# DeepakSridhar/fgdm

Hardware: AMD Instinct MI355X
Metric: 512x512 images/sec @ 50 DDIM steps, seg-ControlNet+CFG (higher is better)
Workload: dtype f16

## Files before the change

fgdm_amd/_lib.py:

```python
import ctypes as C
import os

HERE = os.path.dirname(os.path.abspath(__file__))
LIB_PATH = os.path.join(HERE, 'libfgdm_hip.so')

MAX_LEVELS = 8
MAX_CONTROLNETS = 4

FLAG_USE_ORIGINAL = 1
FLAG_ONLY_MID_CONTROL = 2
FLAG_NO_CONTROL = 4
FLAG_CFG_PAIRS = 8

ACT_NONE, ACT_SILU, ACT_RELU, ACT_GEGLU, ACT_QGELU = 0, 1, 2, 3, 4
OUT_F16, OUT_F32, OUT_F32_NCHW, OUT_F16_T = 0, 1, 2, 3
STRIDE2_PAD_BR = -2


class FgdmConfig(C.Structure):
    _fields_ = [
        ('in_channels', C.c_int32), ('out_channels', C.c_int32), ('model_channels', C.c_int32),
        ('num_res_blocks', C.c_int32), ('n_levels', C.c_int32), ('channel_mult', C.c_int32 * MAX_LEVELS),
        ('n_attention_resolutions', C.c_int32), ('attention_resolutions', C.c_int32 * MAX_LEVELS),
        ('num_heads', C.c_int32), ('context_dim', C.c_int32), ('use_adapter', C.c_int32),
# ... 3 lines not shown
        ('clip_layers', C.c_int32), ('clip_width', C.c_int32), ('clip_heads', C.c_int32), ('clip_mlp', C.c_int32),
        ('clip_vocab', C.c_int32), ('clip_max_len', C.c_int32),
        ('n_extra_adapters', C.c_int32),
        ('vae_encoder', C.c_int32),
    ]


class FgdmConfig2(FgdmConfig):
    _fields_ = [('num_head_channels', C.c_int32), ('use_linear_in_transformer', C.c_int32)]


class FgdmDdimParams(C.Structure):
    _fields_ = [('struct_size', C.c_int64)] + [(name, C.c_void_p) for name in (
        'x', 'cond', 'uncond', 'timesteps', 'alphas', 'alphas_prev', 'sqrt_one_minus_alphas', 'control_scales', 'sigmas',
        'cfg_scales', 'step_noise', 'mask', 'x0', 'q_noise', 'sqrt_alphas_cumprod_t', 'sqrt_one_minus_alphas_cumprod_t',
        'log_steps', 'x_inter_out', 'pred_x0_out')] + [('cfg_scale', C.c_float)] + [(name, C.c_int32) for name in (
            'S', 'B', 'H', 'W', 'flags', 'n_log', 'reserved0')]


class FgdmPlmsParams(C.Structure):
    _fields_ = [('struct_size', C.c_int64)] + [(name, C.c_void_p) for name in (
        'x', 'cond', 'uncond', 'timesteps', 'alphas', 'alphas_prev', 'sqrt_one_minus_alphas', 'control_scales', 'mask', 'x0',
        'q_noise', 'sqrt_alphas_cumprod_t', 'sqrt_one_minus_alphas_cumprod_t', 'log_steps', 'x_inter_out', 'pred_x0_out')] + [
            ('cfg_scale', C.c_float)] + [(name, C.c_int32) for name in ('S', 'B', 'H', 'W', 'flags', 'n_log', 'reserved0')]


class FgdmDpmppParams(C.Structure):
    _fields_ = [('struct_size', C.c_int64)] + [(name, C.c_void_p) for name in (
        'x', 'cond', 'uncond', 'control_scales', 't_float', 'inv_alpha', 'neg_sigma_over_alpha', 'update_kind', 'c1', 'cm0',
        'cm1')] + [('cfg_scale', C.c_float)] + [(name, C.c_int32) for name in (
            'n_eval', 'B', 'H', 'W', 'flags', 'reserved0', 'reserved1')]


class FgdmDpmSolverParams(C.Structure):
    _fields_ = [('struct_size', C.c_int64)] + [(name, C.c_void_p) for name in (
        'x', 'cond', 'uncond', 'control_scales', 't_float', 'conv_x', 'conv_e', 'slot', 'nterms', 'plane', 'coef', 'dest')] + [
            ('cfg_scale', C.c_float)] + [(name, C.c_int32) for name in ('n_eval', 'B', 'H', 'W', 'flags', 'reserved0', 'reserved1')]


class FgdmAncestralParams(C.Structure):
    _fields_ = [('struct_size', C.c_int64)] + [(name, C.c_void_p) for name in (
        'x', 'cond', 'timesteps', 'sqrt_recip_alphas_cumprod', 'sqrt_recipm1_alphas_cumprod', 'posterior_mean_coef1',
        'posterior_mean_coef2', 'std', 'step_noise', 'control_scales', 'mask', 'x0', 'q_noise', 'sqrt_alphas_cumprod_t',
        'sqrt_one_minus_alphas_cumprod_t', 'log_steps', 'x_inter_out')] + [(name, C.c_int32) for name in (
            'S', 'B', 'H', 'W', 'flags', 'n_log', 'reserved0', 'reserved1')]


class FgdmDdimEncodeParams(C.Structure):
    _fields_ = [('struct_size', C.c_int64)] + [(name, C.c_void_p) for name in (
        'x', 'cond', 'uncond', 'timesteps', 'cx', 'ce', 'control_scales', 'log_steps', 'x_inter_out')] + [
            ('cfg_scale', C.c_float)] + [(name, C.c_int32) for name in ('S', 'B', 'H', 'W', 'flags', 'n_log', 'reserved0')]


class FgdmAttentionCapture(C.Structure):
    _fields_ = [('struct_size', C.c_int64), ('tokens', C.POINTER(C.c_int32)), ('block_mask', C.c_uint32)] + [
        (name, C.c_int32) for name in ('n_tokens', 'rows', 'mode', 'batch', 'latent_h', 'latent_w', 'reserved0')]


ATTENTION_CAPTURE_MAX_KEYS = 256
CAPTURE_ROWS = {'all': 0, 'cond': 1, 'uncond': 2}
CAPTURE_MODES = {'sum': 0, 'last': 1}
DPMPP_FIRST, DPMPP_SECOND = 1, 2
DPM_PLANE_BASE, DPM_PLANE_HIST0, DPM_PLANE_M, DPM_DEST_STATE, DPM_DEST_EVAL = 0, 1, 4, 1, 2
PLMS_PROBE, PLMS_FINISH_FIRST, PLMS_MULTISTEP = 0, 1, 2

_p = C.c_void_p
_f = C.c_float
_i = C.c_int
_i64 = C.c_int64

SIGNATURES = {
    'fgdm_create': (_i, [C.POINTER(FgdmConfig), _i, C.POINTER(_p)]),
    'fgdm_destroy': (None, [_p]),
    'fgdm_last_error': (C.c_char_p, [_p]),
    'fgdm_param_count': (_i, [C.POINTER(FgdmConfig)]),
    'fgdm_param_info': (_i, [C.POINTER(FgdmConfig), _i, C.c_char_p, _i, C.POINTER(_i64), C.POINTER(_i)]),
    'fgdm_load_tensor': (_i, [_p, C.c_char_p, _p, _i, C.POINTER(_i64), _i]),
    'fgdm_finalize_weights': (_i, [_p]),
    'fgdm_set_hint': (_i, [_p, _i, _p, _i, _i, _i, _p]),
    'fgdm_set_concat': (_i, [_p, _p, _i, _i, _i, _i, _p]),
    'fgdm_set_adapter_conds': (_i, [_p, _p, _i, _i, _i, _i, _p]),
    'fgdm_set_context': (_i, [_p, _p, _i, _p]),
    'fgdm_apply_model': (_i, [_p, _p, _p, _p, _p, _p, _p, _i, _i, _i, _i, _p, _p]),
    'fgdm_clip_encode': (_i, [_p, _p, _i, _i, _p, _p]),
    'fgdm_clip_encode_skip': (_i, [_p, _p, _i, _i, _i, _p, _p]),
    'fgdm_set_context_tokens': (_i, [_p, _i]),
    'fgdm_get_context_tokens': (_i, [_p]),
    'fgdm_attention_capture_set': (_i, [_p, C.POINTER(FgdmAttentionCapture)]),
    'fgdm_attention_capture_reset': (_i, [_p, _p]),
    'fgdm_attention_capture_info': (_i, [_p, _i, C.POINTER(_i64), C.POINTER(C.c_int32)]),
    'fgdm_attention_capture_block_size': (_i, [_p, _i, C.POINTER(C.c_int32), C.POINTER(C.c_int32)]),
    'fgdm_attention_capture_read': (_i, [_p, _i, _p, _p]),
    'fgdm_run_block': (_i, [_p, C.c_char_p, _p, _i, _p, _i, _p, _p, _i, _i, _i, _p, _i64, C.POINTER(_i64), _p]),
    'fgdm_vae_decode': (_i, [_p, _p, _i, _i, _i, _f, _p, _p]),
    'fgdm_vae_encode': (_i, [_p, _p, _i, _i, _i, _p, _p]),
    'fgdm_unfold': (_i, [_p] + [_i] * 10 + [_p, _p]),
    'fgdm_fold_weighted': (_i, [_p, _p, _p] + [_i] * 9 + [_p, _p]),
    'fgdm_vae_decode_patches': (_i, [_p, _p, _i, _i, _i, _f] + [_i] * 5 + [_p, _p, _i, _p, _p]),
    'fgdm_apply_model_patches': (_i, [_p, _p, _p, _p, _p] + [_i] * 7 + [_p, _p, _i, _i, _p, _p]),
    'fgdm_posterior_sample': (_i, [_p, _p, _f, _p, _i, _i, _i, _p]),
    'fgdm_image_to_uint8': (_i, [_p, _i, _i, _i, _i, _i, _p, _p]),
    'fgdm_resize_linear_uint8': (_i, [_p, _i, _i, _i, _i, _i, _i, _p, _p]),
    'fgdm_uint8_to_hint': (_i, [_p, _i, _i, _i, _i, _p, _p]),
    'fgdm_controlnet': (_i, [_p, _i, _p, _p, _p, _i, _i, _i, _p, _i64, _p]),
    'fgdm_ddim_step': (_i, [_p, _p, _p, _f, _f, _f, _f, _f, _p, _p, _p, _p, _i64, _p]),
    'fgdm_plms_combine': (_i, [_p, _p, _p, _p, _i, _p, _i64, _p]),
    'fgdm_axpby': (_i, [_p, _f, _p, _f, _p, _i64, _p]),
    'fgdm_mask_blend': (_i, [_p, _p, _p, _p, _i64, _p]),
    'fgdm_ancestral_step': (_i, [_p, _p, _f, _f, _f, _f, _f, _p, _p, _i64, _p]),
    'fgdm_sample_ddim': (_i, [_p, _p, _p, _p, _f, _i, C.POINTER(_i64), C.POINTER(_f), C.POINTER(_f), C.POINTER(_f),
                              _p, _i, _i, _i, _i, _p]),
    'fgdm_sample_ddim_ex': (_i, [_p, C.POINTER(FgdmDdimParams), _p]),
    'fgdm_op_ddim_loop_step': (_i, [_p, _p, _p, _f, _f, _f, _f, _f, _p, _p, _p, _p, _f, _f, _p, _p, _p, _p, _p, _i64, _p]),
    'fgdm_sample_plms': (_i, [_p, C.POINTER(FgdmPlmsParams), _p]),
    'fgdm_sample_dpmpp': (_i, [_p, C.POINTER(FgdmDpmppParams), _p]),
    'fgdm_op_plms_loop_step': (_i, [_p, _p, _p, _f, _i, _i, _p, _p, _p, _p, _f, _f, _f, _p, _p, _p, _f, _f, _p, _p, _p, _p, _p,
                                    _i64, _p]),
    'fgdm_op_dpmpp_loop_step': (_i, [_p, _p, _p, _f, _f, _f, _p, _i, _f, _f, _f, _p, _p, _p, _p, _i64, _p]),
    'fgdm_sample_dpm_solver': (_i, [_p, C.POINTER(FgdmDpmSolverParams), _p]),
    'fgdm_op_dpm_program_step': (_i, [_p, _p, _p, _f, _f, _f, _p, _p, _p, _p, _i, _i, _p, _p, _p, _p, _p, _i64, _p]),
    'fgdm_sample_ancestral': (_i, [_p, C.POINTER(FgdmAncestralParams), _p]),
    'fgdm_ddim_encode': (_i, [_p, C.POINTER(FgdmDdimEncodeParams), _p]),
    'fgdm_op_ancestral_loop_step': (_i, [_p, _p, _f, _f, _f, _f, _f, _p, _p, _p, _p, _f, _f, _p, _p, _p, _i64, _p]),
    'fgdm_op_invert_loop_step': (_i, [_p, _p, _p, _f, _f, _f, _p, _p, _p, _p, _i64, _p]),
    'fgdm_profile_begin': (_i, [_p, _i]),
    'fgdm_profile_end': (_i, [_p, C.POINTER(C.c_double)]),
    'fgdm_workspace_stats': (_i, [_p, C.POINTER(_i64), C.POINTER(_i64)]),
    'fgdm_launch_stats': (_i, [_p, C.POINTER(_i64), C.POINTER(_i64), C.POINTER(_i64)]),
    'fgdm_replay_plan': (_i, [_i, _p, _p, _p, _p, _i, _i, _p, _i, _p]),
    'fgdm_op_conv2d': (_i, [_p, _i, _p, _i, _p, _p, _p, _p, _i, _i, _i, _i, _i, _i, _i, _i, _f, _p, _p]),
    'fgdm_op_linear': (_i, [_p, _p, _p, _p, _i, _i, _i, _i, _i, _i, _i, _p, _p]),
    'fgdm_debug_force_igemm_cfg': (_i, [_i]),
    'fgdm_bench_igemm': (_i, [_i] * 13 + [C.POINTER(_f)]),
    'fgdm_op_linear_ln_linear': (_i, [_p] * 8 + [_i] * 5 + [_p, _p, C.POINTER(_i), _p]),
    'fgdm_bench_norm': (_i, [_i] * 7 + [C.POINTER(_f)]),
    'fgdm_bench_attention': (_i, [_i] * 6 + [C.POINTER(_f)]),
    'fgdm_bench_attention_maps': (_i, [_i] * 7 + [C.POINTER(_f)]),
    'fgdm_bench_ff': (_i, [_i] * 4 + [C.POINTER(_f)]),
    'fgdm_op_groupnorm': (_i, [_p, _i, _p, _i, _i, _i, _p, _p, _f, _i, _p, _p]),
    'fgdm_op_layernorm': (_i, [_p, _i, _i, _p, _p, _f, _p, _p]),
    'fgdm_op_attention': (_i, [_p, _i, _p, _i, _p, _i, _p, _i, _i, _i, _i, _i, _i, _p]),
    'fgdm_op_attention_ex': (_i, [_p, _i, _p, _i, _p, _i, _p, _i, _i, _i, _i, _i, _i, _i, _p]),
    'fgdm_debug_last_attention_kernel': (_i, []),
    'fgdm_op_cross_attention_maps': (_i, [_p, _i, _p, _i, _p, _i, _p, _i, _p, _i, _i, _i, _i, _i, _i, _p]),
    'fgdm_op_small_attention': (_i, [_p, _i, _i, _i, _p, _i, _i, _i, _i, _i, _i, _p]),
    'fgdm_op_vae_attention': (_i, [_p, _p, _p, _p, _i, _i, _i, _p]),
    'fgdm_op_softmax_rows': (_i, [_p, _p, _i, _i, _p]),
    'fgdm_op_nchw_to_nhwc': (_i, [_p, _p, _i, _i, _i, _i, _p]),
    'fgdm_op_nhwc_to_nchw': (_i, [_p, _p, _i, _i, _i, _p]),
    'fgdm_op_pack_xcat': (_i, [_p, _p, _i, _i, _i, _i, _i, _i, _p, _p]),
    'fgdm_op_avgpool2': (_i, [_p, _p, _i, _i, _i, _i, _p]),
    'fgdm_op_transpose_pad': (_i, [_p, _p, _i, _i, _i, _i, _p]),
    'fgdm_op_timestep_embed': (_i, [_p, _p, _p, _i, _i, _i, _p]),
    'fgdm_op_add_f16': (_i, [_p, _p, _p, _i64, _p]),
    'fgdm_op_ln_qkv': (_i, [_p] * 6 + [_i] * 5 + [_p, _p, _p]),
}

_lib = None


def load():
    global _lib
    if _lib is not None:
        return _lib
    try:
        import torch
# ... 14 lines not shown
```

fgdm_amd/csrc/engine.hip:

```cpp
#include "model.h"
#include "knobs.h"
#include "replay.h"

#include <algorithm>
#include <array>
#include <cmath>
#include <cstdlib>
#include <cstdio>
#include <cstring>
#include <map>
#include <memory>
#include <string>
#include <unordered_map>
#include <vector>

namespace {

struct Arena {
    struct Blk { char* p; size_t sz; bool free; };
    std::vector<std::vector<Blk>> slabs;
    std::vector<char*> bases;
    size_t slab_bytes = (size_t)4 << 30;
    size_t in_use = 0, peak = 0;
    bool scoped = false;
    std::vector<void*> live;
    void begin_scope() { scoped = true; live.clear(); }
    void end_scope(bool failed) {
        if (failed) { std::vector<void*> l; l.swap(live); scoped = false; for (void* p : l) release(p); }
        scoped = false;
        live.clear();
    }

    ~Arena() { for (char* b : bases) (void)hipFree(b); }
    void* alloc(size_t bytes) {
        bytes = (bytes + 255) & ~(size_t)255;
        if (bytes == 0) bytes = 256;
        for (auto& s : slabs)
            for (size_t i = 0; i < s.size(); ++i)
                if (s[i].free && s[i].sz >= bytes) {
                    if (s[i].sz > bytes) {
                        Blk rest{s[i].p + bytes, s[i].sz - bytes, true};
                        s[i].sz = bytes;
                        s.insert(s.begin() + i + 1, rest);
                    }
                    s[i].free = false;
                    in_use += bytes;
                    peak = std::max(peak, in_use);
                    if (scoped) live.push_back(s[i].p);
                    return s[i].p;
                }
        const size_t sz = std::max(slab_bytes, bytes);
        char* base = nullptr;
        if (hipMalloc(&base, sz) != hipSuccess) return nullptr;
        bases.push_back(base);
        slabs.push_back({Blk{base, sz, true}});
        return alloc(bytes);
    }
    void release(void* p) {
        if (!p) return;
        if (scoped) { auto it = std::find(live.begin(), live.end(), p); if (it != live.end()) { *it = live.back(); live.pop_back(); } }
        for (auto& s : slabs)
            for (size_t i = 0; i < s.size(); ++i)
                if (s[i].p == p && !s[i].free) {
                    s[i].free = true;
                    in_use -= s[i].sz;
                    if (i + 1 < s.size() && s[i + 1].free) { s[i].sz += s[i + 1].sz; s.erase(s.begin() + i + 1); }
                    if (i > 0 && s[i - 1].free) { s[i - 1].sz += s[i].sz; s.erase(s.begin() + i); }
                    return;
                }
    }
};

enum ProfClass { PC_IGEMM = 0, PC_ATTN = 1, PC_NORM = 2, PC_ELEM = 3, PC_COUNT = 4 };
struct Prof final : LaunchTimer {
    bool on = false;
    std::vector<hipEvent_t> pool;
    size_t used = 0;
    struct Rec { int cls; size_t e0, e1; double w; char tag[56]; };
    std::vector<Rec> recs;
    double work[PC_COUNT] = {0, 0, 0, 0};
    double bytes[PC_COUNT] = {0, 0, 0, 0};
    hipEvent_t get() {
        if (used == pool.size()) { hipEvent_t e; if (hipEventCreate(&e) != hipSuccess) return nullptr; pool.push_back(e); }
        return pool[used++];
    }
// ... 39 lines not shown
    struct CtxKV { Tensor k, vt; };
    std::unordered_map<const Layer*, CtxKV> ctx_cache;
    int ctx_B = 0, ctx_T = 0;
    int ctx_tokens = 77;
    struct CapPlane { int block = 0, heads = 0, h = 0, w = 0; float* acc = nullptr; };
    struct Capture {
        bool on = false, capturing = false;
        int rows_sel = 0, mode = 0, Tk = 0;
        int B = 0, H = 0, W = 0;
        int row0 = 0, rows = 0, n_evals = 0;
        std::vector<int> tokens;
        int* tok_dev = nullptr;
        float* head_planes = nullptr;
        std::vector<const Layer*> order;
        std::unordered_map<const Layer*, CapPlane> planes;
    } cap;
    void capture_free() {
        for (auto& kv : cap.planes) { (void)hipFree(kv.second.acc); kv.second.acc = nullptr; }
        (void)hipFree(cap.tok_dev); (void)hipFree(cap.head_planes);
        cap.tok_dev = nullptr; cap.head_planes = nullptr;
        cap.B = cap.H = cap.W = 0;
    }
    void capture_off() { capture_free(); cap = Capture{}; }
    size_t capture_plane_floats(const CapPlane& p) const { return (size_t)cap.rows * p.h * p.w * cap.tokens.size(); }
    int capture_alloc(int B, int H, int W) {
        capture_free();
        const bool half = cap.rows_sel != FGDM_CAPTURE_ROWS_ALL;
        if (half && (B & 1)) return fail(FGDM_ERR_STATE, "attention capture: the conditional / unconditional half of an odd batch");
        cap.rows = half ? B / 2 : B;
        cap.row0 = cap.rows_sel == FGDM_CAPTURE_ROWS_COND ? B / 2 : 0;
        int h = H, w = W;
        size_t scratch = 0;
        auto walk = [&](const Block& blk) -> int {
            for (const Layer& l : blk) {
                if (l.type == L_DOWN) { h = (h + 1) / 2; w = (w + 1) / 2; }
                if (l.type == L_UP) { h *= 2; w *= 2; }
                auto it = l.type == L_ATTN ? cap.planes.find(&l) : cap.planes.end();
                if (it == cap.planes.end()) continue;
                CapPlane& p = it->second;
                p.h = h; p.w = w; p.heads = l.heads;
                scratch = std::max(scratch, attention_capture_plane_floats(B, l.heads, h * w, cap.Tk));
            }
            return FGDM_OK;
        };
        CHK0(for_each_block(unet, false, walk));
        bool ok = hipMalloc(&cap.tok_dev, cap.tokens.size() * sizeof(int)) == hipSuccess &&
                  hipMemcpy(cap.tok_dev, cap.tokens.data(), cap.tokens.size() * sizeof(int), hipMemcpyHostToDevice) == hipSuccess &&
                  hipMalloc(&cap.head_planes, scratch * sizeof(float)) == hipSuccess;
        for (auto& kv : cap.planes) {
            const size_t bytes = capture_plane_floats(kv.second) * sizeof(float);
            ok = ok && hipMalloc(&kv.second.acc, bytes) == hipSuccess && hipMemset(kv.second.acc, 0, bytes) == hipSuccess;
        }
        if (!ok) { capture_free(); return fail(FGDM_ERR_NOMEM, "hipMalloc (attention capture)"); }
        cap.B = B; cap.H = H; cap.W = W;
        cap.n_evals = 0;
        return FGDM_OK;
    }
    int capture_begin(int B, int H, int W) {
        if (cap.Tk != ctx_tokens) return fail(FGDM_ERR_STATE, "attention capture: the context token count changed after the plan was set");
        if (!cap.B) CHK0(capture_alloc(B, H, W));
        if (B != cap.B || H != cap.H || W != cap.W)
            return fail(FGDM_ERR_STATE, "attention capture: this evaluation's batch or latent size is not the one the accumulators were made for");
        cap.capturing = true;
        ++cap.n_evals;
        return FGDM_OK;
    }
    Tensor ccat;
    Arena arena;
    half_t* zero = nullptr;
    int cur_comp = -1;
    bool ln_fold = true;
    hipStream_t s = nullptr;
    std::vector<std::unique_ptr<Arena>> cn_arena;
    Arena* ar = &arena;
    hipStream_t s2 = nullptr;
    hipEvent_t ev_fork = nullptr, ev_join = nullptr;
    bool twin_streams = false;
    bool pair_launch = true;
    int group_max = FGDM_MAX_GROUP;
    bool gn_group = true;
    ReplayStats replay_stats;
    struct Deferred { const GemmW* w; Tensor src; int idx; float scale; Arena* owner; };
    Prof prof;

    const ParamSlot* slot(const std::string& name) {
        auto it = params.find(name);
        if (it == params.end() || !it->second.loaded) { err = "parameter not loaded: " + name; return nullptr; }
        return &it->second;
    }
    template <typename T> T* upload(const std::vector<T>& h) {
        T* d = nullptr;
        if (hipMalloc(&d, std::max<size_t>(h.size() * sizeof(T), 256)) != hipSuccess) return nullptr;
        if (hipMemcpy(d, h.data(), h.size() * sizeof(T), hipMemcpyHostToDevice) != hipSuccess) return nullptr;
        comps[cur_comp].allocs.push_back(d);
        return d;
    }
    int pack_rows(GemmW& g, const std::vector<std::pair<const float*, int>>& srcs, int K_src, int K,
                  const std::vector<int>& kmap, const std::vector<const float*>& biases, bool geglu,
                  const std::vector<float>& src_scale = {}, const float* ln_gamma = nullptr, const float* ln_beta = nullptr) {
        int N = 0;
        for (auto& s : srcs) N += s.second;
        const size_t npad = igemm_npad(N);
        std::vector<half_t> w(npad * (size_t)K, (half_t)0);
        std::vector<float> bias(npad, 0.f), lnu(ln_gamma ? npad : 0, 0.f);
        std::vector<const float*> rowp(N);
        std::vector<float> bflat(N, 0.f), rscale(N, 1.f);
        int r = 0;
        for (size_t si = 0; si < srcs.size(); ++si)
            for (int i = 0; i < srcs[si].second; ++i, ++r) {
                rowp[r] = srcs[si].first + (size_t)i * K_src;
                if (si < biases.size() && biases[si]) bflat[r] = biases[si][i];
                if (si < src_scale.size()) rscale[r] = src_scale[si];
            }
        for (int pr = 0; pr < N; ++pr) {
            int sr = pr;
            if (geglu) {
                const int grp = pr >> 6, within = pr & 63;
                sr = within < 32 ? grp * 32 + within : N / 2 + grp * 32 + (within - 32);
            }
            const float* src = rowp[sr];
            const float rs = rscale[sr];
            half_t* dst = w.data() + (size_t)pr * K;
            if (ln_gamma) {
                double us = 0.0, cs = 0.0;
                for (int k = 0; k < K; ++k) {
                    dst[k] = (half_t)(src[k] * rs * ln_gamma[k]);
                    us += (double)(float)dst[k];
                    cs += (double)ln_beta[k] * (double)(src[k] * rs);
                }
                lnu[pr] = (float)us;
                bias[pr] = (float)((double)(bflat[sr] * rs) + cs);
                continue;
            }
            if (kmap.empty()) for (int k = 0; k < K; ++k) dst[k] = (half_t)(src[k] * rs);
            else for (int k = 0; k < K; ++k) if (kmap[k] >= 0) dst[k] = (half_t)(src[kmap[k]] * rs);
            bias[pr] = bflat[sr] * rs;
        }
        g.N = N; g.K = K; g.k_real = K_src;
        g.w = upload(w);
        g.bias = upload(bias);
        g.ln_u = ln_gamma ? upload(lnu) : nullptr;
        if (ln_gamma && !kmap.empty()) return fail(FGDM_ERR_ARG, "LayerNorm fold: plain Linear weights only");
        return (g.w && g.bias && (!ln_gamma || g.ln_u)) ? FGDM_OK : fail(FGDM_ERR_NOMEM, "hipMalloc failed while packing weights");
    }
    int pack_linear(GemmW& g, const std::string& pre, bool has_bias, bool geglu = false, float wscale = 1.f,
                    const std::string& ln = std::string()) {
        const ParamSlot* w = slot(pre + ".weight");
        if (!w) return FGDM_ERR_STATE;
        const ParamSlot *lg = nullptr, *lb = nullptr;
        if (!ln.empty()) { lg = slot(ln + ".weight"); lb = slot(ln + ".bias"); if (!lg || !lb) return FGDM_ERR_STATE; }
        const ParamSlot* b = has_bias ? slot(pre + ".bias") : nullptr;
        if (has_bias && !b) return FGDM_ERR_STATE;
        const int N = (int)w->shape[0], K = (int)(w->numel() / w->shape[0]);
        if (K & 63) return fail(FGDM_ERR_ARG, "linear K not a multiple of 64: " + pre);
        if (lg && (int)lg->numel() != K) return fail(FGDM_ERR_ARG, "LayerNorm fold: width mismatch for " + pre);
        return pack_rows(g, {{w->host.data(), N}}, K, K, {}, {b ? b->host.data() : nullptr}, geglu, {wscale},
                         lg ? lg->host.data() : nullptr, lb ? lb->host.data() : nullptr);
    }
    int pack_stack(GemmW& g, const std::vector<std::string>& pres, bool has_bias, const std::vector<float>& scales = {},
                   const std::string& ln = std::string()) {
        const ParamSlot *lg = nullptr, *lb = nullptr;
        if (!ln.empty()) { lg = slot(ln + ".weight"); lb = slot(ln + ".bias"); if (!lg || !lb) return FGDM_ERR_STATE; }
        std::vector<std::pair<const float*, int>> srcs;
        std::vector<const float*> biases;
        int K = 0;
        for (auto& pre : pres) {
// ... 382 lines not shown
          int rc;
          auto cp = cap.capturing ? cap.planes.find(&l) : cap.planes.end();
          if (cp != cap.planes.end()) {
              const CapPlane& p = cp->second;
              if (B != cap.B || T != p.h * p.w || Tk != cap.Tk) return fail(FGDM_ERR_STATE, "attention capture: block shape differs from the plan's");
              rc = attention_capture_launch(q2.p, C, k2.p, C, v2t.p, Tkp, a.p, C, B, l.heads, T, Tk, d, 1, cap.head_planes, s);
              if (rc == FGDM_OK)
                  rc = attention_maps_reduce(cap.head_planes, p.acc, l.heads, T, Tk, cap.row0, cap.rows, cap.tok_dev, (int)cap.tokens.size(),
                                             cap.mode == FGDM_CAPTURE_SUM, s);
          } else {
              rc = attention_launch(q2.p, C, k2.p, C, v2t.p, Tkp, a.p, C, B, l.heads, T, Tk, d, 1, s);
          }
          prof.end(s);
          if (rc != FGDM_OK) return fail(rc, "attention launch failed"); }
        tfree(q2);
        if (!cached) { tfree(k2); tfree(v2t); }
        { Epi e; e.resid = h2.p; e.ld_res = C; if (ln_fold) e.stats = &s3; CHK(linear(l.o2, a, e, &h)); }
        tfree(a); tfree(h2);
        if (!ln_fold) CHK(lnorm(l.ln3, h, &nrm));
        { Epi e; if (ln_fold) e.ln = &s3; e.act = ACT_GEGLU; CHK(linear(l.ffp, ln_fold ? h : nrm, e, &f)); }
        if (s3.p) ar->release(s3.p);
        if (nrm.p) tfree(nrm);
        { Epi e; e.resid = h.p; e.ld_res = C; CHK(linear(l.ffo, f, e, &h2)); }
        tfree(f); tfree(h);
        { Epi e; e.resid = x.p; e.ld_res = C; CHK(linear(l.pout, h2, e, out)); }
        tfree(h2);
        if (x_full.p) tfree(x_full);
        return FGDM_OK;
    }

    int dup_rows(const Tensor& h, Tensor* full) {
        *full = talloc(2 * h.B, h.H, h.W, h.C);
        if (!full->p) return fail(FGDM_ERR_NOMEM, "workspace");
        const size_t bytes = h.numel() * sizeof(half_t);
        CHK(dcopy(full->p, h.p, bytes));
        CHK(dcopy((char*)full->p + bytes, h.p, bytes));
        return FGDM_OK;
    }
    int block_fwd_shared(const Block& blk, Tensor xh, bool own_x, const EmbCtx& ec, const Tensor& ctx16, Tensor* out) {
        Tensor cur = xh;
        bool own = own_x, full = false;
        for (size_t j = 0; j < blk.size(); ++j) {
            const Layer& l = blk[j];
            Tensor nxt;
            switch (l.type) {
                case L_CONV: CHK(conv3(l.conv, cur, nullptr, 1, false, Epi{}, &nxt)); break;
                case L_RES: CHK(res_fwd(l, cur, nullptr, ec, &nxt)); break;
                case L_ATTN: CHK(attn_fwd(l, cur, ctx16, &nxt, !full)); full = true; break;
                case L_DOWN: CHK(conv3(l.conv, cur, nullptr, 2, false, Epi{}, &nxt)); break;
                case L_UP: CHK(conv3(l.conv, cur, nullptr, 1, true, Epi{}, &nxt)); break;
            }
            if (own) tfree(cur);
            cur = nxt;
            own = true;
        }
        if (!full) { Tensor f; CHK(dup_rows(cur, &f)); if (own) tfree(cur); cur = f; }
        *out = cur;
        return FGDM_OK;
    }

    int block_fwd(const Block& blk, Tensor x, bool own_x, const Tensor* x1, const EmbCtx& ec, const Tensor& ctx16,
                  const half_t* conv_resid, Tensor* out) {
        Tensor cur = x;
        bool own = own_x;
        for (size_t j = 0; j < blk.size(); ++j) {
            const Layer& l = blk[j];
            Tensor nxt;
            switch (l.type) {
                case L_CONV: { Epi e; if (conv_resid) { e.resid = conv_resid; e.ld_res = l.cout; }
                               CHK(conv3(l.conv, cur, nullptr, 1, false, e, &nxt)); break; }
                case L_RES: CHK(res_fwd(l, cur, j == 0 ? x1 : nullptr, ec, &nxt)); break;
                case L_ATTN: CHK(attn_fwd(l, cur, ctx16, &nxt)); break;
                case L_DOWN: CHK(conv3(l.conv, cur, nullptr, 2, false, Epi{}, &nxt)); break;
                case L_UP: CHK(conv3(l.conv, cur, nullptr, 1, true, Epi{}, &nxt)); break;
            }
            if (own) tfree(cur);
            cur = nxt;
            own = true;
        }
        *out = cur;
        return FGDM_OK;
    }

    int embed(Net& n, const int64_t* t, const float* tf, int B, float** emb_all) {
        const int mc = cfg.model_channels;
        Tensor te = talloc(1, 1, B, mc), e1, e2;
        if (!te.p) return fail(FGDM_ERR_NOMEM, "workspace");
        if (timestep_embed(t, tf, te.p, B, mc, B, s) != FGDM_OK) return fail(FGDM_ERR_HIP, "timestep_embed");
        { Epi e; e.act = ACT_SILU; e.rps = 1; CHK(linear(n.time0, te, e, &e1)); }
        { Epi e; e.act = ACT_SILU; e.rps = 1; CHK(linear(n.time2, e1, e, &e2)); }
        *emb_all = (float*)ar->alloc((size_t)B * n.emb_total * sizeof(float));
        if (!*emb_all) return fail(FGDM_ERR_NOMEM, "workspace");
        { Epi e; e.out_kind = OUT_F32; e.out = *emb_all; e.ld_out = n.emb_total; e.rps = 1; CHK(linear(n.emb_all, e2, e, nullptr)); }
        tfree(te); tfree(e1); tfree(e2);
        return FGDM_OK;
    }

    int adapter_fwd(Net& n, const Tensor& x4, Tensor feats[4]) { return adapter_run(n.ad_conv_in, n.ad_body, x4, feats); }
    int adapter_run(const GemmW& conv_in, const std::vector<AdapterBlk>& body, const Tensor& x4, Tensor feats[4]) {
        Tensor cur;
        CHK(conv3(conv_in, x4, nullptr, 1, false, Epi{}, &cur));
        auto drop = [&](Tensor& t) {
            for (int f = 0; f < 4; ++f) if (feats[f].p == t.p) return;
            tfree(t);
        };
        for (size_t k = 0; k < body.size(); ++k) {
            const AdapterBlk& b = body[k];
            if (b.down) {
                Tensor p = talloc(cur.B, cur.H / 2, cur.W / 2, cur.C);
                if (!p.p) return fail(FGDM_ERR_NOMEM, "workspace");
                if (avgpool2(cur.p, p.p, cur.B, cur.H, cur.W, cur.C, s) != FGDM_OK)
                    return fail(FGDM_ERR_ARG, "avgpool2: latent size must be divisible by 8 for the adapter");
                drop(cur);
                cur = p;
            }
            if (b.ic != b.oc) { Tensor y; CHK(linear(b.in_conv, cur, Epi{}, &y)); drop(cur); cur = y; }
            Tensor h, y;
            { Epi e; e.act = ACT_RELU; CHK(conv3(b.b1, cur, nullptr, 1, false, e, &h)); }
            { Epi e; e.resid = cur.p; e.ld_res = cur.C; CHK(linear(b.b2, h, e, &y)); }
            tfree(h);
            drop(cur);
            cur = y;
            if (k % 2 == 1) feats[k / 2] = cur;
        }
        return FGDM_OK;
    }

    void drop_adapter_conds() {
        for (Tensor& t : unet.xad_sum) { if (t.p) (void)hipFree(t.p); t = Tensor{}; }
        unet.xad_valid = false;
    }
    int set_adapter_conds(const float* const* conds, int nc, int B, int H, int W) {
        if (!finalized) return fail(FGDM_ERR_STATE, "weights not finalized");
        Net& n = unet;
        drop_adapter_conds();
        if (nc == 0) return FGDM_OK;
        if (nc < 0 || nc > (int)n.xad_body.size() || !conds) return fail(FGDM_ERR_ARG, "more conds than extra adapters (n_extra_adapters)");
        if (B <= 0 || (H & 7) || (W & 7)) return fail(FGDM_ERR_ARG, "latent size must be divisible by 8 for the adapter");
        for (int kk = 0; kk < nc; ++kk) {
            Tensor c4 = talloc(B, H, W, 4), f[4];
            if (!c4.p) return fail(FGDM_ERR_NOMEM, "workspace");
            if (nchw_f32_to_nhwc_f16(conds[kk], c4.p, B, 4, H * W, 4, s) != FGDM_OK) return fail(FGDM_ERR_HIP, "layout kernel");
            CHK(adapter_run(n.xad_conv_in[kk], n.xad_body[kk], c4, f));
            tfree(c4);
            for (int i = 0; i < 4; ++i) {
                Tensor& acc = n.xad_sum[i];
                if (kk == 0) {
                    acc = f[i];
                    if (hipMalloc(&acc.p, acc.numel() * sizeof(half_t)) != hipSuccess) return fail(FGDM_ERR_NOMEM, "hipMalloc (adapter cache)");
                    HIP_TRY(hipMemcpyAsync(acc.p, f[i].p, acc.numel() * sizeof(half_t), hipMemcpyDeviceToDevice, s));
                } else if (add_f16(acc.p, f[i].p, acc.p, acc.numel(), s) != FGDM_OK) {
                    return fail(FGDM_ERR_HIP, "add kernel");
                }
                tfree(f[i]);
            }
        }
        n.xad_valid = true;
        return FGDM_OK;
    }

    int time_adapter_fwd(Net& n, const Tensor& x4, const EmbCtx& ec, Tensor feats[4]) {
        Tensor cur;
        CHK(conv3(n.ad_conv_in, x4, nullptr, 1, false, Epi{}, &cur));
        for (size_t k = 0; k < n.tad_body.size(); ++k) {
            Tensor y;
            CHK(res_fwd(n.tad_body[k], cur, nullptr, ec, &y));
            bool keep = false;
            for (int f = 0; f < 4; ++f) if (feats[f].p == cur.p) keep = true;
            if (!keep) tfree(cur);
            cur = y;
            if (k % 2 == 1) feats[k / 2] = cur;
        }
        return FGDM_OK;
    }

    int run_block(const std::string& prefix, const float* x, int C, const float* x_skip, int Cs, const float* emb,
                  const float* ctx, int B, int H, int W, float* out, int64_t cap, int64_t* out_numel) {
        if (!finalized) return fail(FGDM_ERR_STATE, "weights not finalized");
        if (B <= 0 || H <= 0 || W <= 0 || C <= 0) return fail(FGDM_ERR_ARG, "bad shape");
// ... 60 lines not shown
            if (f32_to_f16(ctx, ctx16.p, ctx16.numel(), s) != FGDM_OK) return fail(FGDM_ERR_HIP, "convert kernel");
        }
        float* emb_all = nullptr;
        if (needs_emb) {
            const int temb = 4 * cfg.model_channels;
            Tensor e2 = talloc(1, 1, B, temb);
            emb_all = (float*)ar->alloc((size_t)B * net->emb_total * sizeof(float));
            if (!e2.p || !emb_all) return fail(FGDM_ERR_NOMEM, "workspace");
            if (silu_f32_to_f16(emb, e2.p, e2.numel(), s) != FGDM_OK) return fail(FGDM_ERR_HIP, "silu kernel");
            { Epi e; e.out_kind = OUT_F32; e.out = emb_all; e.ld_out = net->emb_total; e.rps = 1; CHK(linear(net->emb_all, e2, e, nullptr)); }
            tfree(e2);
        }
        EmbCtx ec{emb_all, net->emb_total};
        Tensor y;
        CHK(block_fwd(*blk, xin, false, x_skip ? &xsk : nullptr, ec, ctx16, nullptr, &y));
        CHK(emit(y, off));
        tfree(y); tfree(xin);
        if (xsk.p) tfree(xsk);
        if (ctx16.p) tfree(ctx16);
        if (emb_all) ar->release(emb_all);
        if (out_numel) *out_numel = off;
        return FGDM_OK;
    }

    int ensure_device() {
        if (device_ready) return FGDM_OK;
        if (hipSetDevice(device) != hipSuccess) return fail(FGDM_ERR_HIP, "hipSetDevice failed (no GPU?)");
        if (hipMalloc(&zero, 4096) != hipSuccess || hipMemset(zero, 0, 4096) != hipSuccess) return fail(FGDM_ERR_HIP, "hipMalloc failed");
        if (cfg.workspace_bytes > 0) arena.slab_bytes = (size_t)cfg.workspace_bytes;
        device_ready = true;
        return FGDM_OK;
    }

    int zero_conv_into(const GemmW& zw, const Tensor& src, Tensor& dst, float scale) {
        Epi e;
        e.scale = scale;
        if (src.B * 2 == dst.B) {
            for (int half = 0; half < 2; ++half) {
                half_t* d = dst.p + (size_t)half * (dst.numel() / 2);
                e.resid = d; e.ld_res = dst.C; e.out = d; e.ld_out = dst.C;
                CHK(linear(zw, src, e, nullptr));
            }
            return FGDM_OK;
        }
        e.resid = dst.p; e.ld_res = dst.C; e.out = dst.p; e.ld_out = dst.C;
        return linear(zw, src, e, nullptr);
    }

    struct RecordScope {
        fgdm_engine& e;
        Arena* const ar0;
        RecWalk* const rec0;
        RecordScope(fgdm_engine& e_, RecWalk* walk, Arena* arena) : e(e_), ar0(e_.ar), rec0(fgdm_record_into(walk)) { e.ar = arena; }
        ~RecordScope() { e.ar = ar0; fgdm_record_into(rec0); }
        RecordScope(const RecordScope&) = delete;
    };
    bool hint_twins = false;
    int hint_pair = 1;
    struct LayerHints {
        fgdm_engine& e;
        const bool twins0;
        const int pair0;
        LayerHints(fgdm_engine& e_, bool twins, int pair_mult = 0) : e(e_), twins0(e_.hint_twins), pair0(e_.hint_pair) {
            e.set_hints(twins, pair_mult > 0 ? pair_mult : pair0);
        }
        ~LayerHints() { e.set_hints(twins0, pair0); }
        LayerHints(const LayerHints&) = delete;
    };
    void set_hints(bool twins, int pair_mult) {
        igemm_set_twin_layers(hint_twins = twins);
        igemm_set_pair_hint(hint_pair = pair_mult);
    }

    int controlnet_fwd(Net& n, const Tensor& x4, const int64_t* t, const float* tf, const Tensor& ctx16, const float* scales,
                       std::vector<Tensor>* hs, Tensor* h_mid, bool only_mid, float* out32, int64_t out_cap, bool pairs = false,
                       std::vector<Deferred>* defer = nullptr) {
        const int B = x4.B;
        LayerHints twins(*this, true);
        const bool shared = pairs && !out32 && 2 * n.guided.B == B && n.input.size() > 1;
        if (!n.guided.p) return fail(FGDM_ERR_STATE, "fgdm_set_hint has not been called for this ControlNet");
        if (!(n.guided.B == B || 2 * n.guided.B == B) || n.guided.H != x4.H || n.guided.W != x4.W)
            return fail(FGDM_ERR_ARG, "cached hint does not match the batch / latent size");
        float* emb = nullptr;
        CHK(embed(n, t, tf, B, &emb));
        EmbCtx ec{emb, n.emb_total};
        Tensor h;
        int64_t off = 0;
        auto zero_conv = [&](const GemmW& zw, const Tensor& src, int idx) -> int {
            Epi e;
            if (out32) {
                const int64_t cnt = (int64_t)src.numel();
                if (off + cnt > out_cap) return fail(FGDM_ERR_ARG, "fgdm_controlnet: output buffer too small");
                e.out_kind = OUT_F32_NCHW; e.out = out32 + off; e.ld_out = src.H * src.W;
                off += cnt;
                return linear(zw, src, e, nullptr);
            }
            if (idx >= 0 && only_mid) return FGDM_OK;
            e.scale = scales ? scales[idx < 0 ? (int)n.input.size() : idx] : 1.f;
            if (defer) { defer->push_back({&zw, src, idx, e.scale, ar}); return FGDM_OK; }
            return zero_conv_into(zw, src, idx < 0 ? *h_mid : (*hs)[idx], e.scale);
        };
        for (size_t i = 0; i < n.input.size(); ++i) {
            Tensor nxt;
            if (i == 0) {
                const Layer& l = n.input[0][0];
                if (shared) {
                    Tensor xh = x4; xh.B = B / 2;
                    CHK(block_fwd(n.input[0], xh, false, nullptr, ec, ctx16, n.guided.p, &nxt));
                } else if (n.guided.B == B) {
                    CHK(block_fwd(n.input[0], x4, false, nullptr, ec, ctx16, n.guided.p, &nxt));
                } else {
                    nxt = talloc(B, x4.H, x4.W, l.cout);
                    if (!nxt.p) return fail(FGDM_ERR_NOMEM, "workspace");
                    for (int half = 0; half < 2; ++half) {
                        Tensor xs = x4; xs.B = B / 2; xs.p = x4.p + (size_t)half * xs.numel();
                        Epi e; e.resid = n.guided.p; e.ld_res = l.cout;
                        e.out = nxt.p + (size_t)half * (nxt.numel() / 2); e.ld_out = l.cout;
                        CHK(conv3(l.conv, xs, nullptr, 1, false, e, nullptr));
                    }
                }
            } else if (shared && i == 1) {
                CHK(block_fwd_shared(n.input[1], h, !defer, ec, ctx16, &nxt));
            } else {
                CHK(block_fwd(n.input[i], h, !defer, nullptr, ec, ctx16, nullptr, &nxt));
            }
            h = nxt;
            CHK(zero_conv(n.zero_convs[i], h, (int)i));
        }
        Tensor m;
        CHK(block_fwd(n.middle, h, !defer, nullptr, ec, ctx16, nullptr, &m));
        CHK(zero_conv(n.mid_out, m, -1));
        if (!defer) tfree(m);
        ar->release(emb);
        return FGDM_OK;
    }

    template <class PerNet>
    int controlnets_fwd(const Tensor& x4, const int64_t* t, const float* tf, const Tensor& ctx16, const float* scales, std::vector<Tensor>* hs,
                        Tensor* h_mid, bool only_mid, bool pairs, std::vector<Deferred>* defer, PerNet per_net) {
        for (size_t c = 0; c < cns.size(); ++c) {
            RecordScope scope = per_net(c);
            CHK(controlnet_fwd(cns[c], x4, t, tf, ctx16, scales ? scales + 13 * c : nullptr, hs, h_mid, only_mid, nullptr, 0, pairs, defer));
        }
        return FGDM_OK;
    }

    int apply_model(const float* x, const int64_t* t, const float* tf, const float* ctx, const float* pcond,
                    const float* scales, int B, int H, int W, int flags, float* eps_out) {
        if (!cap.on) return apply_model_walk(x, t, tf, ctx, pcond, scales, B, H, W, flags, eps_out);
        if (!finalized) return fail(FGDM_ERR_STATE, "weights not finalized");
        if (B <= 0 || H <= 0 || W <= 0) return fail(FGDM_ERR_ARG, "bad shape");
        CHK(capture_begin(B, H, W));
        const int rc = apply_model_walk(x, t, tf, ctx, pcond, scales, B, H, W, flags, eps_out);
        cap.capturing = false;
        return rc;
    }
    int apply_model_walk(const float* x, const int64_t* t, const float* tf, const float* ctx, const float* pcond,
                         const float* scales, int B, int H, int W, int flags, float* eps_out) {
        if (!finalized) return fail(FGDM_ERR_STATE, "weights not finalized");
        if (B <= 0 || H <= 0 || W <= 0) return fail(FGDM_ERR_ARG, "bad shape");
        Net& n = unet;
        const int HW = H * W;
        const int Cc = cfg.in_channels - 4;
        if (Cc > 0) {
            if (!ccat.p) return fail(FGDM_ERR_STATE, "in_channels > 4 but no c_concat was registered (fgdm_set_concat)");
            if (!(ccat.B == B || (B % 2 == 0 && 2 * ccat.B == B)))
                return fail(FGDM_ERR_STATE, "the registered c_concat has " + std::to_string(ccat.B) + " rows: the batch must have as many, or twice as many");
            if (ccat.H != H || ccat.W != W) return fail(FGDM_ERR_STATE, "the registered c_concat has another latent size than x");
        }
        Tensor x4 = talloc(B, H, W, Cc > 0 ? n.input[0][0].conv.cin_pad : 4), ctx16;
        if (ctx) ctx16 = talloc(B, 1, ctx_tokens, cfg.context_dim);
        else if (ctx_B != B) return fail(FGDM_ERR_STATE, "ctx is NULL but no context of this batch size was registered (fgdm_set_context)");
        if (!x4.p || (ctx && !ctx16.p)) return fail(FGDM_ERR_NOMEM, "workspace");
        const bool pairs = (flags & FGDM_FLAG_CFG_PAIRS) && (B % 2 == 0) && n.input.size() > 1;
        if (Cc > 0) {
            const int rows = pairs ? B / 2 : B;
            if (pack_xcat(x, ccat.p, x4.p, rows, std::min(ccat.B, rows), Cc, HW, x4.C, s) != FGDM_OK) return fail(FGDM_ERR_HIP, "pack kernel");
        } else if (nchw_f32_to_nhwc_f16(x, x4.p, B, 4, HW, 4, s) != FGDM_OK) return fail(FGDM_ERR_HIP, "layout kernel");
        if (ctx && f32_to_f16(ctx, ctx16.p, ctx16.numel(), s) != FGDM_OK) return fail(FGDM_ERR_HIP, "convert kernel");
        float* emb = nullptr;
        CHK(embed(n, t, tf, B, &emb));
        EmbCtx ec{emb, n.emb_total};

        const bool use_adapter = n.has_adapter && !(flags & FGDM_FLAG_USE_ORIGINAL);
        const int Bs = pairs ? B / 2 : B;
        Tensor x4s = x4; x4s.B = Bs;
        Tensor fa[4];
        if (use_adapter) {
            if (pcond) {
                Tensor p4 = talloc(Bs, H, W, 4);
                if (!p4.p) return fail(FGDM_ERR_NOMEM, "workspace");
                if (nchw_f32_to_nhwc_f16(pcond, p4.p, Bs, 4, HW, 4, s) != FGDM_OK) return fail(FGDM_ERR_HIP, "layout kernel");
                CHK(n.time_adapter ? time_adapter_fwd(n, p4, ec, fa) : adapter_fwd(n, p4, fa));
                tfree(p4);
            } else {
                CHK(n.time_adapter ? time_adapter_fwd(n, x4s, ec, fa) : adapter_fwd(n, x4s, fa));
            }
        }
        const bool with_cn = !cns.empty() && !(flags & FGDM_FLAG_NO_CONTROL);
        const bool twin = twin_streams && with_cn && s2 && !(flags & FGDM_FLAG_ONLY_MID_CONTROL);
        std::vector<Deferred> deferred;
        const bool paired = pair_launch && with_cn && !twin && !(flags & FGDM_FLAG_ONLY_MID_CONTROL);
        std::vector<Tensor> hs;
        Tensor h, hm;
        auto encoder = [&]() -> int {
            LayerHints twins(*this, with_cn);
            int k = 0;
            Tensor h0s;
            for (size_t i = 0; i < n.input.size(); ++i) {
                Tensor nxt;
                if (pairs && i == 0) {
                    CHK(block_fwd(n.input[0], x4s, false, nullptr, ec, ctx16, nullptr, &h0s));
                    CHK(dup_rows(h0s, &nxt));
                } else if (pairs && i == 1) {
                    CHK(block_fwd_shared(n.input[1], h0s, true, ec, ctx16, &nxt));
                } else {
                    CHK(block_fwd(n.input[i], i == 0 ? x4 : h, false, nullptr, ec, ctx16, nullptr, &nxt));
                }
                if (use_adapter && (i + 1) % 3 == 0) {
                    if (k >= 4 || fa[k].numel() * (size_t)(B / Bs) != nxt.numel()) return fail(FGDM_ERR_ARG, "adapter feature shape mismatch (latent size must be divisible by 8)");
                    for (int half = 0; half < B / Bs; ++half) {
                        half_t* dst = nxt.p + (size_t)half * fa[k].numel();
                        if (n.xad_valid) {
                            if (n.xad_sum[k].numel() != nxt.numel()) return fail(FGDM_ERR_ARG, "registered adapter conds do not match this batch / latent size");
                            const half_t* xs = n.xad_sum[k].p + (size_t)half * fa[k].numel();
                            if (add_f16(dst, xs, dst, fa[k].numel(), s) != FGDM_OK) return fail(FGDM_ERR_HIP, "add kernel");
                        }
                        if (add_f16(dst, fa[k].p, dst, fa[k].numel(), s) != FGDM_OK) return fail(FGDM_ERR_HIP, "add kernel");
                    }
                    tfree(fa[k]);
                    ++k;
                }
                h = nxt;
                hs.push_back(h);
            }
            CHK(block_fwd(n.middle, h, false, nullptr, ec, ctx16, nullptr, &hm));
            return FGDM_OK;
        };
        if (paired) {
            std::vector<RecWalk> walks(1 + cns.size());
            {
                const bool fat = knob_once(KNOB_PAIR_FAT_TILES) != 0;
                LayerHints fused(*this, false, fat ? std::min<int>(group_max, 1 + (int)cns.size()) : 0);
                groupnorm_set_group(gn_group);
                CHK(controlnets_fwd(x4, t, tf, ctx16, scales, nullptr, nullptr, false, pairs, &deferred,
                                    [&](size_t c) { return RecordScope(*this, &walks[1 + c], cn_arena[c].get()); }));
                RecordScope rec(*this, &walks[0], &arena);
                CHK(encoder());
            }
            std::vector<RecWalk*> lists;
            for (RecWalk& w : walks) lists.push_back(&w);
            CHK(fgdm_replay(lists, group_max, s, prof, replay_stats));
        } else {
            if (twin) {
                if (hipEventRecord(ev_fork, s) != hipSuccess || hipStreamWaitEvent(s2, ev_fork, 0) != hipSuccess) return fail(FGDM_ERR_HIP, "stream fork");
                hipStream_t main_s = s;
                s = s2;
                const int rc = controlnets_fwd(x4, t, tf, ctx16, scales, nullptr, nullptr, false, pairs, &deferred,
                                               [&](size_t) { return RecordScope(*this, nullptr, cn_arena[0].get()); });
                s = main_s;
                if (rc != FGDM_OK) return rc;
                if (hipEventRecord(ev_join, s2) != hipSuccess) return fail(FGDM_ERR_HIP, "stream join");
            }
            CHK(encoder());
        }
        if (twin || paired) {
            if (twin && hipStreamWaitEvent(s, ev_join, 0) != hipSuccess) return fail(FGDM_ERR_HIP, "stream join");
            for (const Deferred& d : deferred) CHK(zero_conv_into(*d.w, d.src, d.idx < 0 ? hm : hs[d.idx], d.scale));
            for (Deferred& d : deferred) { d.owner->release(d.src.p); d.src.p = nullptr; }
        } else if (with_cn) {
            CHK(controlnets_fwd(x4, t, tf, ctx16, scales, &hs, &hm, (flags & FGDM_FLAG_ONLY_MID_CONTROL) != 0, pairs, nullptr,
                                [&](size_t) { return RecordScope(*this, nullptr, &arena); }));
        }
        h = hm;
        for (size_t i = 0; i < n.output.size(); ++i) {
            Tensor skip = hs.back();
            hs.pop_back();
            Tensor nxt;
            CHK(block_fwd(n.output[i], h, true, &skip, ec, ctx16, nullptr, &nxt));
            tfree(skip);
            h = nxt;
        }
        Tensor g;
        CHK(gnorm(n.out_gn, h, nullptr, 1e-5f, true, &g));
        tfree(h);
        { Epi e; e.out_kind = OUT_F32_NCHW; e.out = eps_out; e.ld_out = HW; CHK(conv3(n.out_conv, g, nullptr, 1, false, e, nullptr)); }
        tfree(g);
        tfree(x4);
        if (ctx16.p) tfree(ctx16);
        ar->release(emb);
        return FGDM_OK;
    }

    int clip_encode(const int64_t* ids, int B, int T, float* out, int clip_skip = 0) {
        if (!clip.on) return fail(FGDM_ERR_STATE, "engine was created without a text encoder (clip_layers = 0)");
        if (!comps[clip_comp].packed) return fail(FGDM_ERR_STATE, "weights not finalized");
        if (B <= 0 || T <= 0 || T > cfg.clip_max_len) return fail(FGDM_ERR_ARG, "bad shape (T must be <= clip_max_len)");
        if (clip_skip > cfg.clip_layers + 1) return fail(FGDM_ERR_ARG, "clip_skip exceeds the number of hidden states");
        const int n_run = cfg.clip_layers - (clip_skip > 1 ? clip_skip - 1 : 0);
        int li = 0;
        const int W = cfg.clip_width, rows = B * T;
        Tensor n, qkv, a, f;
        float* h = (float*)ar->alloc((size_t)rows * W * sizeof(float));
        float* h2 = (float*)ar->alloc((size_t)rows * W * sizeof(float));
        if (!h || !h2) return fail(FGDM_ERR_NOMEM, "workspace");
        if (embed_tokens(ids, clip.tok, clip.pos, h, rows, T, W, cfg.clip_vocab, s) != FGDM_OK) return fail(FGDM_ERR_HIP, "embedding kernel");
        auto ln32 = [&](const NormW& nw, const float* src, Tensor* dst) -> int {
            *dst = talloc(1, 1, rows, W);
            if (!dst->p) return fail(FGDM_ERR_NOMEM, "workspace");
            return layernorm32_launch(src, rows, W, nw.g, nw.b, 1e-5f, dst->p, nullptr, s) == FGDM_OK ? FGDM_OK : fail(FGDM_ERR_HIP, "layernorm");
        };
        for (const ClipLayer& l : clip.layers) {
            if (li++ >= n_run) break;
            CHK(ln32(l.ln1, h, &n));
            CHK(linear(l.qkv, n, Epi{}, &qkv));
            tfree(n);
            a = talloc(1, 1, rows, W);
            if (!a.p) return fail(FGDM_ERR_NOMEM, "workspace");
            if (small_attention_launch(qkv.p, 3 * W, W, 2 * W, a.p, W, B, cfg.clip_heads, T, W / cfg.clip_heads, 1, s) != FGDM_OK)
                return fail(FGDM_ERR_HIP, "text attention kernel");
            tfree(qkv);
            Tensor br;
            CHK(linear(l.o, a, Epi{}, &br));
            tfree(a);
            if (add_f16_to_f32(h, br.p, h2, br.numel(), s) != FGDM_OK) return fail(FGDM_ERR_HIP, "add kernel");
            tfree(br);
            CHK(ln32(l.ln2, h2, &n));
            { Epi e; e.act = ACT_QGELU; CHK(linear(l.fc1, n, e, &f)); }
            tfree(n);
            CHK(linear(l.fc2, f, Epi{}, &br));
            tfree(f);
            if (add_f16_to_f32(h2, br.p, h, br.numel(), s) != FGDM_OK) return fail(FGDM_ERR_HIP, "add kernel");
            tfree(br);
        }
        if (layernorm32_launch(h, rows, W, clip.final_ln.g, clip.final_ln.b, 1e-5f, nullptr, out, s) != FGDM_OK) return fail(FGDM_ERR_HIP, "layernorm");
        ar->release(h); ar->release(h2);
        return FGDM_OK;
    }

    int vattn_fwd(const VAttn& at, const Tensor& x, Tensor* out) {
        const int B = x.B, T = x.H * x.W, C = x.C;
        if (T & 63) return fail(FGDM_ERR_ARG, "first-stage attention: H*W must be a multiple of 64");
        Tensor g, q, k, vt, a, P;
        CHK(gnorm(at.norm, x, nullptr, 1e-6f, false, &g));
        CHK(linear(at.q, g, Epi{}, &q));
        k = talloc(1, 1, B * T + 128, C);
        vt = talloc(B, 1, C, T);
        a = talloc(B, x.H, x.W, C);
        P = talloc(1, 1, T, T);
        float* S = (float*)ar->alloc((size_t)T * T * sizeof(float));
        if (!k.p || !vt.p || !a.p || !P.p || !S) return fail(FGDM_ERR_NOMEM, "workspace");
        HIP_TRY(hipMemsetAsync(k.p + (size_t)B * T * C, 0, (size_t)128 * C * sizeof(half_t), s));
        { Epi e; e.out = k.p; e.ld_out = C; e.rps = T; CHK(linear(at.k, g, e, nullptr)); }
        { Epi e; e.out_kind = OUT_F16_T; e.out = vt.p; e.ld_out = T; e.rps = T; CHK(linear(at.v, g, e, nullptr)); }
        tfree(g);
        bool softmax_failed = false;
        const int rc = vattn_core(q.p, k.p, vt.p, a.p, S, P.p, B, T, C, s, &softmax_failed,
            [&](const half_t* Wt, int N, int K, const half_t* A, int M, int out_kind, void* o, int ld_out, float scale) {
                GemmW w; w.w = const_cast<half_t*>(Wt); w.N = N; w.K = K; w.k_real = K;
                Tensor xa; xa.p = const_cast<half_t*>(A); xa.B = 1; xa.H = 1; xa.W = M; xa.C = K;
                Epi e; e.out_kind = out_kind; e.out = o; e.ld_out = ld_out; e.rps = M; e.scale = scale;
                return gemm(w, IG_LINEAR, xa, nullptr, 1, M, e, nullptr);
            });
        if (rc != FGDM_OK) return softmax_failed ? fail(rc, "softmax kernel") : rc;
        ar->release(S);
        tfree(P); tfree(q); tfree(k); tfree(vt);
        { Epi e; e.resid = x.p; e.ld_res = C; CHK(linear(at.o, a, e, out)); }
        tfree(a);
        return FGDM_OK;
    }
    int vae_decode(const float* z, int B, int H, int W, float scale, float* out) {
        if (!vae.on) return fail(FGDM_ERR_STATE, "engine was created without a first-stage decoder (vae_ch = 0)");
        if (!comps[vae_comp].packed) return fail(FGDM_ERR_STATE, "weights not finalized");
// ... 121 lines not shown

static std::string g_create_err;

static int make_desc(const fgdm_config* cfg, fgdm_engine** out) {
    fgdm_engine* e = new fgdm_engine();
    e->cfg = *cfg;
    const int rc = e->build();
    if (rc != FGDM_OK) { g_create_err = "unsupported configuration: " + e->err; delete e; return rc; }
    *out = e;
    return FGDM_OK;
}

template <typename F> static int scoped_call(fgdm_engine* e, void* stream, F f) {
    e->s = as_stream(stream);
    e->ar = &e->arena;
    e->arena.begin_scope();
    for (auto& a : e->cn_arena) a->begin_scope();
    const int rc = f();
    e->s = as_stream(stream);
    e->ar = &e->arena;
    if (rc != FGDM_OK && e->s2) (void)hipStreamSynchronize(e->s2);
    e->arena.end_scope(rc != FGDM_OK);
    for (auto& a : e->cn_arena) a->end_scope(rc != FGDM_OK);
    return rc;
}

static bool read_params(const void* caller, int64_t size_v1, void* known, size_t size_lib) {
    int64_t size;
    memcpy(&size, caller, sizeof(size));
    if (size < size_v1 || size > (int64_t)size_lib) return false;
    memset(known, 0, size_lib);
    memcpy(known, caller, (size_t)size);
    return true;
}

template <typename T> static int upload_repeated(const T* host, int count, int Bm, T* dev, hipStream_t s) {
    std::vector<T> th((size_t)count * Bm);
    for (int k = 0; k < count; ++k) for (int b = 0; b < Bm; ++b) th[(size_t)k * Bm + b] = host[k];
    HIP_TRY(hipMemcpyAsync(dev, th.data(), th.size() * sizeof(T), hipMemcpyHostToDevice, s));
    HIP_TRY(hipStreamSynchronize(s));
    return FGDM_OK;
}

static bool loop_cfg_on(const float* uncond, float cfg_scale) { return uncond && cfg_scale != 1.0f; }
static int loop_flags(int flags, bool cfg_on) { return cfg_on ? flags | FGDM_FLAG_CFG_PAIRS : flags & ~FGDM_FLAG_CFG_PAIRS; }

struct Loop {
    fgdm_engine* e;
    hipStream_t s;
    float* x;
    const float* control_scales;
    int B, H, W, K, flags;
    bool cfg_on;
    const int32_t* log_steps;
    int n_log;
    float *x2 = nullptr, *eps = nullptr, *c2 = nullptr, *hist = nullptr;
    int64_t* t_int = nullptr;
    float* t_float = nullptr;
    int Bm = 0, logged = 0;
    size_t n = 0;

    template <typename P> Loop(fgdm_engine* e_, hipStream_t s_, const P& p, int K_, bool cfg_on_, int flags_, const int32_t* log_steps_ = nullptr, int n_log_ = 0)
        : e(e_), s(s_), x(p.x), control_scales(p.control_scales), B(p.B), H(p.H), W(p.W), K(K_), flags(flags_), cfg_on(cfg_on_),
          log_steps(log_steps_), n_log(n_log_) {}

    int begin(const float* cond, const float* uncond, const int64_t* times_int, const float* times_float, int hist_planes) {
        Bm = cfg_on ? 2 * B : B;
        n = (size_t)B * 4 * H * W;
        const size_t nctx = (size_t)B * e->ctx_tokens * e->cfg.context_dim;
        x2 = (float*)e->arena.alloc(Bm * 4 * (size_t)H * W * sizeof(float));
        eps = (float*)e->arena.alloc(Bm * 4 * (size_t)H * W * sizeof(float));
        c2 = (float*)e->arena.alloc(Bm * (size_t)e->ctx_tokens * e->cfg.context_dim * sizeof(float));
        if (!x2 || !eps || !c2) return e->fail(FGDM_ERR_NOMEM, "workspace");
        if (cfg_on) {
            HIP_TRY(hipMemcpyAsync(c2, uncond, nctx * sizeof(float), hipMemcpyDeviceToDevice, s));
            HIP_TRY(hipMemcpyAsync(c2 + nctx, cond, nctx * sizeof(float), hipMemcpyDeviceToDevice, s));
        } else {
            HIP_TRY(hipMemcpyAsync(c2, cond, nctx * sizeof(float), hipMemcpyDeviceToDevice, s));
        }
        CHK(e->set_context(c2, Bm));
        if (hist_planes) hist = (float*)e->arena.alloc(hist_planes * n * sizeof(float));
        void* tdev = e->arena.alloc((size_t)K * Bm * (times_int ? sizeof(int64_t) : sizeof(float)));
        if (!tdev || (hist_planes && !hist)) return e->fail(FGDM_ERR_NOMEM, "workspace");
        if (times_int) return upload_repeated(times_int, K, Bm, t_int = (int64_t*)tdev, s);
        return upload_repeated(times_float, K, Bm, t_float = (float*)tdev, s);
    }
    float* plane(int j) const { return hist + (size_t)j * n; }
    int seed() {
        HIP_TRY(hipMemcpyAsync(x2, x, n * sizeof(float), hipMemcpyDeviceToDevice, s));
        if (cfg_on) HIP_TRY(hipMemcpyAsync(x2 + n, x, n * sizeof(float), hipMemcpyDeviceToDevice, s));
        return FGDM_OK;
    }
    int eval(int k) {
        return e->apply_model(x2, t_int ? t_int + (size_t)k * Bm : nullptr, t_float ? t_float + (size_t)k * Bm : nullptr, nullptr, nullptr,
                              control_scales, Bm, H, W, flags, eps);
    }
    void feed(StepIO& io) const { io.xin_a = x2; io.xin_b = cfg_on ? x2 + n : nullptr; }
    StepIO step_io(int i, float cfg) const {
        StepIO io{};
        io.x = x; io.n = n; io.ec = cfg_on ? eps + n : eps; io.eu = cfg_on ? eps : nullptr; io.cfg = cfg; io.x_out = x;
        if (i + 1 < K) feed(io);
        return io;
    }
    int log_slot(int i) { return logged < n_log && log_steps[logged] == i ? logged++ : -1; }
    float* log_plane(float* out, int slot) const { return out && slot >= 0 ? out + (size_t)slot * n : nullptr; }
    int end(int rc) {
        e->arena.release(x2); e->arena.release(eps); e->arena.release(c2); e->arena.release(hist);
        e->arena.release(t_int); e->arena.release(t_float);
        return rc;
    }
};

static std::string why_text(const char* why) { return why ? why : ""; }
static std::string why_text(const std::string& why) { return why; }
template <typename P, typename Check, typename Body>
static int loop_entry(fgdm_engine* e, const P* caller, void* stream, int64_t size_v1, const char* entry, const char* struct_name,
                      bool refuse_hybrid, Check check, Body body) {
    if (!e || !caller) return FGDM_ERR_ARG;
    const std::string name = entry;
    P known;
    if (!read_params(caller, size_v1, &known, sizeof(known)))
        return e->fail(FGDM_ERR_ARG, name + ": struct_size is not the sizeof(" + struct_name + ") of a known header version");
    const std::string why = why_text(check(known));
    if (!why.empty()) return e->fail(FGDM_ERR_ARG, name + ": " + why);
    if (refuse_hybrid && e->cfg.in_channels > 4) return e->fail(FGDM_ERR_ARG, name + ": in_channels > 4 (hybrid c_concat) is not taken by the device loops");
    if (!e->finalized) return e->fail(FGDM_ERR_STATE, "weights not finalized");
    return scoped_call(e, stream, [&] { return body(e, known, as_stream(stream)); });
}

extern "C" {

int fgdm_create(const fgdm_config* cfg, int device, fgdm_engine** out) {
    if (!cfg || !out) return FGDM_ERR_ARG;
    fgdm_engine* e = nullptr;
    int rc = make_desc(cfg, &e);
    if (rc != FGDM_OK) return rc;
    e->device = device;
    e->ln_fold = knob_on(KNOB_LN_FOLD);
    rc = e->ensure_device();
    if (rc != FGDM_OK) {
        g_create_err = e->err + " [" + hipGetErrorString(hipGetLastError()) + "]";
        delete e;
        return rc;
    }
    e->twin_streams = knob_on(KNOB_TWIN_STREAMS);
    e->pair_launch = knob_on(KNOB_PAIR_LAUNCH);
    e->group_max = std::max(2, std::min(FGDM_MAX_GROUP, knob_int(KNOB_GROUP_MAX)));
    e->gn_group = knob_on(KNOB_GN_GROUP);
    if (e->twin_streams && !e->cns.empty()) {
        if (hipStreamCreateWithFlags(&e->s2, hipStreamNonBlocking) != hipSuccess ||
            hipEventCreateWithFlags(&e->ev_fork, hipEventDisableTiming) != hipSuccess ||
            hipEventCreateWithFlags(&e->ev_join, hipEventDisableTiming) != hipSuccess) {
            g_create_err = "second stream could not be created";
            delete e;
            return FGDM_ERR_HIP;
        }
    }
    for (size_t c = 0; c < e->cns.size(); ++c) {
        e->cn_arena.emplace_back(new Arena());
        if (e->cfg.workspace_bytes > 0) e->cn_arena.back()->slab_bytes = (size_t)e->cfg.workspace_bytes;
    }
    *out = e;
    return FGDM_OK;
}

void fgdm_destroy(fgdm_engine* e) {
    if (!e) return;
    for (hipEvent_t ev : e->prof.pool) (void)hipEventDestroy(ev);
    for (auto& c : e->comps) for (void* p : c.allocs) (void)hipFree(p);
    if (e->zero) (void)hipFree(e->zero);
    for (auto& n : e->cns) if (n.guided.p) (void)hipFree(n.guided.p);
    e->drop_concat();
    e->drop_context();
    e->drop_adapter_conds();
    e->capture_free();
    if (knob_text(KNOB_PAIR_DEBUG) && e->replay_stats.replayed)
        fprintf(stderr, "[fgdm] grouped twin launches: %ld of %ld replayed launches were fused (%ld problems)\n", e->replay_stats.fused, e->replay_stats.replayed, e->replay_stats.problems);
    if (e->s2) { (void)hipStreamSynchronize(e->s2); (void)hipStreamDestroy(e->s2); }
    if (e->ev_fork) (void)hipEventDestroy(e->ev_fork);
    if (e->ev_join) (void)hipEventDestroy(e->ev_join);
    delete e;
}

const char* fgdm_last_error(const fgdm_engine* e) { return e ? e->err.c_str() : g_create_err.c_str(); }

static fgdm_engine* g_desc = nullptr;
static fgdm_config g_desc_cfg;
static fgdm_engine* desc_for(const fgdm_config* cfg) {
    if (g_desc && memcmp(&g_desc_cfg, cfg, sizeof(*cfg)) == 0) return g_desc;
    if (g_desc) { delete g_desc; g_desc = nullptr; }
    if (make_desc(cfg, &g_desc) != FGDM_OK) return nullptr;
    g_desc_cfg = *cfg;
    return g_desc;
}
int fgdm_param_count(const fgdm_config* cfg) {
    if (!cfg) return FGDM_ERR_ARG;
    fgdm_engine* d = desc_for(cfg);
    return d ? (int)d->order.size() : FGDM_ERR_ARG;
}
int fgdm_param_info(const fgdm_config* cfg, int index, char* name, int name_cap, int64_t* shape, int* ndim) {
    if (!cfg || !name || !shape || !ndim) return FGDM_ERR_ARG;
    fgdm_engine* d = desc_for(cfg);
    if (!d || index < 0 || index >= (int)d->order.size()) return FGDM_ERR_ARG;
    const std::string& n = d->order[index];
    if ((int)n.size() + 1 > name_cap) return FGDM_ERR_ARG;
    memcpy(name, n.c_str(), n.size() + 1);
    const auto& sh = d->params[n].shape;
    *ndim = (int)sh.size();
    for (size_t i = 0; i < sh.size(); ++i) shape[i] = sh[i];
    return FGDM_OK;
}

int fgdm_load_tensor(fgdm_engine* e, const char* key, const void* data, int dtype, const int64_t* shape, int ndim) {
    if (!e || !key || !data || !shape) return FGDM_ERR_ARG;
    auto it = e->params.find(key);
    if (it == e->params.end()) return e->fail(FGDM_ERR_ARG, std::string("unknown parameter key: ") + key);
    ParamSlot& ps = it->second;
    if ((int)ps.shape.size() != ndim) return e->fail(FGDM_ERR_ARG, std::string("rank mismatch for ") + key);
    for (int i = 0; i < ndim; ++i)
        if (ps.shape[i] != shape[i]) return e->fail(FGDM_ERR_ARG, std::string("shape mismatch for ") + key);
    const size_t n = ps.numel();
    ps.host.resize(n);
    if (dtype == FGDM_DTYPE_F32) {
        if (hipMemcpy(ps.host.data(), data, n * sizeof(float), hipMemcpyDefault) != hipSuccess) return e->fail(FGDM_ERR_HIP, "hipMemcpy failed");
    } else if (dtype == FGDM_DTYPE_F16) {
        std::vector<half_t> tmp(n);
        if (hipMemcpy(tmp.data(), data, n * sizeof(half_t), hipMemcpyDefault) != hipSuccess) return e->fail(FGDM_ERR_HIP, "hipMemcpy failed");
        for (size_t i = 0; i < n; ++i) ps.host[i] = (float)tmp[i];
    } else {
        return e->fail(FGDM_ERR_ARG, "unsupported dtype");
    }
    ps.loaded = true;
    e->comps[ps.comp].dirty = true;
    e->finalized = false;
    return FGDM_OK;
}

int fgdm_finalize_weights(fgdm_engine* e) {
    if (!e) return FGDM_ERR_ARG;
    int rc = e->ensure_device();
    if (rc != FGDM_OK) return rc;
    e->drop_context();
    e->drop_adapter_conds();
    for (auto& n : e->cns) if (n.guided.p) { (void)hipFree(n.guided.p); n.guided = Tensor{}; }
    for (int c = 0; c < (int)e->comps.size(); ++c) { rc = e->repack(c); if (rc != FGDM_OK) return rc; }
    e->finalized = true;
    return FGDM_OK;
}

int fgdm_profile_begin(fgdm_engine* e, int stride) {
    if (!e) return FGDM_ERR_ARG;
    e->prof.on = true;
    e->prof.stride = stride > 0 ? stride : 1;
    e->prof.counter = 0;
    e->prof.used = 0;
    e->prof.recs.clear();
    for (int c = 0; c < PC_COUNT; ++c) { e->prof.work[c] = 0; e->prof.bytes[c] = 0; }
    return FGDM_OK;
}
int fgdm_profile_end(fgdm_engine* e, double* out) {
    if (!e || !out) return FGDM_ERR_ARG;
    e->prof.on = false;
    if (hipDeviceSynchronize() != hipSuccess) return e->fail(FGDM_ERR_HIP, "hipDeviceSynchronize failed");
    for (int c = 0; c < PC_COUNT * 4; ++c) out[c] = 0;
    for (auto& r : e->prof.recs) {
        if (!r.e1) continue;
        float ms = 0.f;
        if (hipEventElapsedTime(&ms, e->prof.pool[r.e0], e->prof.pool[r.e1]) != hipSuccess) continue;
        out[r.cls * 4 + 0] += ms;
        out[r.cls * 4 + 1] += 1;
    }
    for (int c = 0; c < PC_COUNT; ++c) { out[c * 4 + 2] = e->prof.work[c]; out[c * 4 + 3] = e->prof.bytes[c]; }
    if (const char* path = knob_text(KNOB_PROF_DUMP)) {
        std::map<std::string, std::array<double, 3>> agg;
        for (auto& r : e->prof.recs) {
            if (!r.e1) continue;
            float ms = 0.f;
            if (hipEventElapsedTime(&ms, e->prof.pool[r.e0], e->prof.pool[r.e1]) != hipSuccess) continue;
            auto& a = agg[r.tag];
            a[0] += 1; a[1] += ms; a[2] += r.w;
        }
        if (FILE* f = fopen(path, "w")) {
            for (auto& kv : agg) fprintf(f, "%s\t%.0f\t%.4f\t%.6g\n", kv.first.c_str(), kv.second[0], kv.second[1], kv.second[2]);
            fclose(f);
        }
    }
    return FGDM_OK;
}
int fgdm_workspace_stats(fgdm_engine* e, int64_t* peak_bytes, int64_t* reserved_bytes) {
    if (!e || !peak_bytes || !reserved_bytes) return FGDM_ERR_ARG;
    size_t pk = e->arena.peak, r = 0;
    for (auto& sl : e->arena.slabs) for (auto& b : sl) r += b.sz;
    for (auto& a : e->cn_arena) {
        pk += a->peak;
        for (auto& sl : a->slabs) for (auto& b : sl) r += b.sz;
    }
    *peak_bytes = (int64_t)pk;
    *reserved_bytes = (int64_t)r;
    return FGDM_OK;
}

int fgdm_launch_stats(fgdm_engine* e, int64_t* replayed_launches, int64_t* fused_launches, int64_t* fused_problems) {
    if (!e || !replayed_launches || !fused_launches || !fused_problems) return FGDM_ERR_ARG;
    *replayed_launches = (int64_t)e->replay_stats.replayed;
    *fused_launches = (int64_t)e->replay_stats.fused;
    *fused_problems = (int64_t)e->replay_stats.problems;
    return FGDM_OK;
}

int fgdm_set_hint(fgdm_engine* e, int cn, const float* hint, int B, int Hh, int Wh, void* stream) {
    if (!e || !hint) return FGDM_ERR_ARG;
    return scoped_call(e, stream, [&] { return e->set_hint(cn, hint, B, Hh, Wh); });
}

int fgdm_set_concat(fgdm_engine* e, const float* c_concat, int B, int Cc, int H, int W, void* stream) {
    if (!e) return FGDM_ERR_ARG;
    return scoped_call(e, stream, [&] { return e->set_concat(c_concat, B, Cc, H, W); });
}

int fgdm_apply_model(fgdm_engine* e, const float* x, const int64_t* t, const float* t_float, const float* ctx,
                     const float* pcond, const float* control_scales, int B, int H, int W, int flags, float* eps_out,
                     void* stream) {
    if (!e || !x || (!t && !t_float) || !eps_out) return FGDM_ERR_ARG;
    return scoped_call(e, stream, [&] { return e->apply_model(x, t, t_float, ctx, pcond, control_scales, B, H, W, flags, eps_out); });
}

int fgdm_set_adapter_conds(fgdm_engine* e, const float* const* conds, int n_conds, int B, int H, int W, void* stream) {
    if (!e) return FGDM_ERR_ARG;
    return scoped_call(e, stream, [&] { return e->set_adapter_conds(conds, n_conds, B, H, W); });
}

int fgdm_set_context(fgdm_engine* e, const float* ctx, int B, void* stream) {
    if (!e || !ctx) return FGDM_ERR_ARG;
    return scoped_call(e, stream, [&] { return e->set_context(ctx, B); });
}

int fgdm_clip_encode(fgdm_engine* e, const int64_t* ids, int B, int T, float* out, void* stream) {
    if (!e || !ids || !out) return FGDM_ERR_ARG;
    return scoped_call(e, stream, [&] { return e->clip_encode(ids, B, T, out); });
}

int fgdm_clip_encode_skip(fgdm_engine* e, const int64_t* ids, int B, int T, int clip_skip, float* out, void* stream) {
    if (!e || !ids || !out) return FGDM_ERR_ARG;
    return scoped_call(e, stream, [&] { return e->clip_encode(ids, B, T, out, clip_skip); });
}

int fgdm_set_context_tokens(fgdm_engine* e, int tokens) {
    if (!e) return FGDM_ERR_ARG;
    if (tokens < 1) return e->fail(FGDM_ERR_ARG, "context token count must be >= 1");
    if (tokens != e->ctx_tokens) { e->drop_context(); e->ctx_tokens = tokens; }
    return FGDM_OK;
}

int fgdm_get_context_tokens(const fgdm_engine* e) { return e ? e->ctx_tokens : FGDM_ERR_ARG; }

int fgdm_attention_capture_set(fgdm_engine* e, const fgdm_attention_capture* plan) {
    if (!e) return FGDM_ERR_ARG;
    if (!plan) { e->capture_off(); return FGDM_OK; }
    fgdm_attention_capture p;
    if (!read_params(plan, FGDM_ATTENTION_CAPTURE_SIZE_V1, &p, sizeof(p)))
        return e->fail(FGDM_ERR_ARG, "attention capture: struct_size is not the sizeof(fgdm_attention_capture) of a known header version");
    if (p.reserved0) return e->fail(FGDM_ERR_ARG, "attention capture: reserved0 must be 0");
    if (!e->finalized) return e->fail(FGDM_ERR_STATE, "weights not finalized");
    std::vector<const Layer*> order;
    for_each_block(e->unet, false, [&](const Block& blk) {
        for (const Layer& l : blk) if (l.type == L_ATTN) order.push_back(&l);
        return FGDM_OK;
    });
    const int nb = (int)order.size(), Tk = e->ctx_tokens;
    if (!p.block_mask || (nb < 32 && (p.block_mask >> nb)))
        return e->fail(FGDM_ERR_ARG, "attention capture: block_mask must name at least one of the UNet's " + std::to_string(nb) + " transformer blocks and no other");
    if (Tk > FGDM_ATTENTION_CAPTURE_MAX_KEYS)
        return e->fail(FGDM_ERR_ARG, "attention capture: the context has " + std::to_string(Tk) + " tokens, more than FGDM_ATTENTION_CAPTURE_MAX_KEYS, the capturing kernels' key limit");
    if (Tk >= 128 && Tk % 64 == 0)
        return e->fail(FGDM_ERR_ARG, "attention capture: a context of 128, 192 or 256 tokens runs on the self-attention kernels, which have no capturing form");
    if (p.n_tokens < 0 || p.n_tokens > Tk || (p.n_tokens > 0 && !p.tokens))
        return e->fail(FGDM_ERR_ARG, "attention capture: n_tokens must lie in [0, context tokens], with tokens given when it is not 0");
    std::vector<int> tokens;
    for (int i = 0; i < (p.n_tokens ? p.n_tokens : Tk); ++i) {
        const int k = p.n_tokens ? p.tokens[i] : i;
        if (k < 0 || k >= Tk) return e->fail(FGDM_ERR_ARG, "attention capture: token index " + std::to_string(k) + " is outside the registered context of " + std::to_string(Tk) + " tokens");
        tokens.push_back(k);
    }
    if (p.rows < FGDM_CAPTURE_ROWS_ALL || p.rows > FGDM_CAPTURE_ROWS_UNCOND) return e->fail(FGDM_ERR_ARG, "attention capture: rows must be FGDM_CAPTURE_ROWS_ALL, _COND or _UNCOND");
    if (p.mode != FGDM_CAPTURE_SUM && p.mode != FGDM_CAPTURE_LAST) return e->fail(FGDM_ERR_ARG, "attention capture: mode must be FGDM_CAPTURE_SUM or FGDM_CAPTURE_LAST");
    const bool sized = p.batch > 0 && p.latent_h > 0 && p.latent_w > 0;
    if (!sized && (p.batch || p.latent_h || p.latent_w))
        return e->fail(FGDM_ERR_ARG, "attention capture: batch, latent_h and latent_w must be all positive or all 0");
    if (sized && p.rows != FGDM_CAPTURE_ROWS_ALL && (p.batch & 1))
        return e->fail(FGDM_ERR_ARG, "attention capture: the conditional / unconditional half of an odd batch");
    e->capture_off();
    auto& c = e->cap;
    c.rows_sel = p.rows; c.mode = p.mode; c.Tk = Tk;
    c.tokens = tokens; c.order = order;
    for (int i = 0; i < nb; ++i)
        if ((p.block_mask >> i) & 1) { fgdm_engine::CapPlane pl; pl.block = i; c.planes[order[i]] = pl; }
    if (sized) {
        const int rc = e->capture_alloc(p.batch, p.latent_h, p.latent_w);
        if (rc != FGDM_OK) { e->capture_off(); return rc; }
    }
    c.on = true;
    return FGDM_OK;
}
static const fgdm_engine::CapPlane* capture_block(fgdm_engine* e, int block) {
    if (!e->cap.on || block < 0 || block >= (int)e->cap.order.size()) return nullptr;
    auto it = e->cap.planes.find(e->cap.order[block]);
    return it == e->cap.planes.end() ? nullptr : &it->second;
// ... 487 lines not shown
```

fgdm_amd/csrc/knobs.h:

```cpp
#pragma once
#include "common.h"
#include <array>
#include <cstdlib>

#define FGDM_STR_(x) #x
#define FGDM_STR(x) FGDM_STR_(x)

#define FGDM_KNOBS(X)                                                                                                          \
    X(ATTN_PP, "FGDM_ATTN_PP", "1", "0: the four-wave attention kernel where the eight-wave ping-pong one would run")           \
    X(ATTN_DQ, "FGDM_ATTN_DQ", "3", "long self-attention, d = 40: 3 = two-strand kernel, 32-wide V^T P^T; 1 = 16-wide; 0 = off") \
    X(ATTN_DQ80, "FGDM_ATTN_DQ80", "1", "0: the ping-pong kernel instead of the two-strand one at d = 64 / 80")                 \
    X(ATTN_ABL, "FGDM_ATTN_ABL", "0", "ablation instantiations of the two-strand kernel (tools/bench_attention.py only)")       \
    X(ATTN_CROSS, "FGDM_ATTN_CROSS", "4", "query chunks per wave of the text-token kernel (65 - 96 keys); 0 = off")             \
    X(ATTN_CROSS_LONG, "FGDM_ATTN_CROSS_LONG", "8", "query chunks per wave of the key-resident kernel (97 - 256 keys); 0 = off") \
    X(IGEMM_EPI_PATHS, "FGDM_IGEMM_EPI_PATHS", "1", "0: the general GEMM epilogue instead of the host-selected straight-line paths") \
    X(IGEMM_HALO, "FGDM_IGEMM_HALO", "1", "0: per-tap K loop instead of the halo-tile loop (stride-1 3x3 convolutions, split K too)") \
    X(IGEMM_MFMA32, "FGDM_IGEMM_MFMA32", "0", "1: automatic tile choices take the 32x32x16 MFMA instantiations")                \
    X(IGEMM_OTHER_WIDTHS, "FGDM_IGEMM_OTHER_WIDTHS", "1", "0: widths 128 / 256 / 512 back on the 2-stage kernel")               \
    X(IGEMM_PERSIST, "FGDM_IGEMM_PERSIST", "1", "GEGLU projections: 1 = persistent, tiles round-robin; 2 = contiguous runs; 0 = off") \
    X(IGEMM_PIPE, "FGDM_IGEMM_PIPE", "1", "0: the phase-locked K loop instead of the software-pipelined one")                   \
    X(IGEMM_UP_PHASE, "FGDM_IGEMM_UP_PHASE", "1", "0: Upsample convs as the 3x3 walk over the virtual upsampled image, not four 2x2 phase GEMMs") \
    X(IGEMM_SMALL_M, "FGDM_IGEMM_SMALL_M", "1", "0: linears with a thin 128-row grid stay on 128 x 320 tiles")                  \
    X(IGEMM_SMALL_TILES, "FGDM_IGEMM_SMALL_TILES", "1", "0: the 8x8 level's linears back on the 2-stage kernel")                \
    X(IGEMM_STATS64, "FGDM_IGEMM_STATS64", "1", "0: the 64 x 160 tile leaves the LayerNorm partial sums to the row-statistics pass") \
    X(SPLITK_FAT, "FGDM_SPLITK_FAT", "1", "0: split K four ways on 128 x 320 tiles at the 8x8 level only")                      \
    X(PAIR_FAT_TILES, "FGDM_PAIR_FAT_TILES", "1", "0: grouped launches keep the tile a single problem would take")              \
    X(GN_REG, "FGDM_GN_REG", "1024", "largest pixel count per sample of the register-resident GroupNorm; 0 = off")              \
    X(GN_REG_NG, "FGDM_GN_REG_NG", "4", "widest slice of the register-resident GroupNorm, in groups")                           \
    X(GN_FUSED_MAXKB, "FGDM_GN_FUSED_MAXKB", "64", "largest LDS slice (KB) of the single-kernel GroupNorm; 0 = always two kernels") \
    X(GN_CHUNK, "FGDM_GN_CHUNK", FGDM_STR(GN_PIX_PER_CHUNK), "pixels per partial-sum chunk of the two-kernel GroupNorm (multiples of 64)") \
    X(LN_FOLD, "FGDM_LN_FOLD", "1", "fgdm_create; 0: the transformer blocks' LayerNorms as kernels of their own")               \
    X(TWIN_STREAMS, "FGDM_TWIN_STREAMS", "0", "fgdm_create; 1: the ControlNets on a second stream next to the UNet encoder")    \
    X(PAIR_LAUNCH, "FGDM_PAIR_LAUNCH", "1", "fgdm_create; 0: no grouped launches of twin layers")                               \
    X(GROUP_MAX, "FGDM_GROUP_MAX", FGDM_STR(FGDM_MAX_GROUP), "fgdm_create; problems per grouped launch, clamped to [2, FGDM_MAX_GROUP]") \
    X(GN_GROUP, "FGDM_GN_GROUP", "1", "fgdm_create; 0: single-pass GroupNorm launches stay out of the grouped launches")        \
    X(PAIR_DEBUG, "FGDM_PAIR_DEBUG", nullptr, "set (to anything): fgdm_destroy prints how many replayed launches were fused")   \
    X(PROF_DUMP, "FGDM_PROF_DUMP", nullptr, "path: fgdm_profile_end writes the per-shape time table there")                     \
    X(BENCH_DATA_SCALE, "FGDM_BENCH_DATA_SCALE", "1", "atof; scale of the random operands of fgdm_bench_igemm / _attention")

enum Knob {
#define X(id, name, dflt, meaning) KNOB_##id,
    FGDM_KNOBS(X)
#undef X
    KNOB_COUNT
};
struct KnobDef { const char* name; const char* dflt; const char* meaning; };
inline constexpr KnobDef KNOB_TABLE[KNOB_COUNT] = {
#define X(id, name, dflt, meaning) {name, dflt, meaning},
    FGDM_KNOBS(X)
#undef X
};

inline const char* knob_text(Knob k) {
    const char* v = getenv(KNOB_TABLE[k].name);
    return v ? v : KNOB_TABLE[k].dflt;
}
inline int knob_int(Knob k) { return atoi(knob_text(k)); }
inline bool knob_on(Knob k) { return knob_int(k) != 0; }
inline int knob_once(Knob k) {
    static const std::array<int, KNOB_COUNT> v = [] {
        std::array<int, KNOB_COUNT> a{};
        for (int i = 0; i < KNOB_COUNT; ++i)
            if (KNOB_TABLE[i].dflt) a[i] = knob_int((Knob)i);
        return a;
    }();
    return v[k];
}
```

fgdm_amd/csrc/ops_abi.hip:

```cpp
#include "engine_shared.h"
#include "replay_plan.h"

static int op_pack(IgemmArgs& a, TmpDev& tmp, const float* w, const float* bias, int N, int K, int Ks, bool geglu,
                   const int* kmap = nullptr, const float* gamma = nullptr, const float* beta = nullptr) {
    auto host = [](const float* d, size_t n, std::vector<float>& v) { v.resize(n); return hipMemcpy(v.data(), d, n * sizeof(float), hipMemcpyDefault) == hipSuccess; };
    std::vector<float> wh, bh(N, 0.f), g, bt;
    if (!host(w, (size_t)N * Ks, wh) || (bias && !host(bias, N, bh))) return FGDM_ERR_HIP;
    if (gamma && (!host(gamma, K, g) || !host(beta, K, bt))) return FGDM_ERR_HIP;
    const size_t npad = igemm_npad(N);
    std::vector<half_t> pk(npad * (size_t)K, (half_t)0);
    std::vector<float> bp(npad, 0.f), u(gamma ? npad : 0, 0.f);
    for (int pr = 0; pr < N; ++pr) {
        int sr = pr;
        if (geglu) { const int grp = pr >> 6, within = pr & 63; sr = within < 32 ? grp * 32 + within : N / 2 + grp * 32 + (within - 32); }
        const float* row = &wh[(size_t)sr * Ks];
        double us = 0.0, cs = 0.0;
        for (int k = 0; k < K; ++k) {
            const int ks = kmap ? kmap[k] : k;
            if (ks < 0) continue;
            const half_t wq = (half_t)(gamma ? row[ks] * g[k] : row[ks]);
            pk[(size_t)pr * K + k] = wq;
            if (gamma) { us += (double)(float)wq; cs += (double)bt[k] * (double)row[ks]; }
        }
        bp[pr] = gamma ? (float)((double)bh[sr] + cs) : bh[sr];
        if (gamma) u[pr] = (float)us;
    }
    a.Wt = tmp.up(pk); a.bias = tmp.up(bp);
    if (gamma) a.ln_u = tmp.up(u);
    return a.Wt && a.bias && (!gamma || a.ln_u) ? FGDM_OK : FGDM_ERR_NOMEM;
}

static int op_gemm_rows(IgemmArgs& a, const half_t* A, int B, int Ho, int Wo, int K, int rps, TmpDev& tmp, hipStream_t s) {
    a.A0 = A; a.C0 = K; a.A1 = nullptr; a.C1 = 0;
    a.zero = g_zero_page();
    if (!a.zero) return FGDM_ERR_NOMEM;
    a.B = B; a.H = Ho; a.W = Wo; a.Ho = Ho; a.Wo = Wo;
    a.M = B * Ho * Wo; a.K = K; a.mode = IG_LINEAR; a.rows_per_sample = rps;
    if (plan_splitk(a, tmp) != FGDM_OK) return FGDM_ERR_NOMEM;
    return igemm_launch(a, s);
}

static int op_conv3_im2col(const half_t* x, int Cin, const float* w, const float* bias, const float* rowvec, const half_t* resid,
                           int B, int H, int W, int Cout, int stride, int act, float scale, void* out, hipStream_t s) {
    int cp = 0;
    const std::vector<int> kmap = conv3_kmap(Cin, &cp);
    const int K = (int)kmap.size(), Ho = (H - 1) / stride + 1, Wo = (W - 1) / stride + 1;
    TmpDev tmp;
    IgemmArgs a{};
    const int prc = op_pack(a, tmp, w, bias, Cout, K, Cin * 9, false, kmap.data());
    if (prc != FGDM_OK) return prc;
    half_t* A = tmp.alloc<half_t>((size_t)B * Ho * Wo * K);
    if (!A) return FGDM_ERR_NOMEM;
    a.rowvec = rowvec; a.rv_stride = Cout;
    a.resid = resid; a.ld_res = Cout;
    a.N = Cout; a.act = act; a.out_kind = OUT_F16; a.out = out; a.ld_out = Cout; a.scale = scale;
    const int rc = im2col_conv(x, A, B, H, W, cp, stride, K, s, []() {},
        [&](half_t* Ap, int Bv, int Hv, int Wv, int Kv, int rps) { return op_gemm_rows(a, Ap, Bv, Hv, Wv, Kv, rps, tmp, s); });
    (void)hipStreamSynchronize(s);
    return rc;
}

extern "C" {

int fgdm_op_conv2d(const void* x0, int C0, const void* x1, int C1, const float* w, const float* bias, const float* rowvec,
                   const void* resid, int B, int H, int W, int Cout, int ksize, int stride, int upsample, int act,
                   float scale, void* out, void* stream) {
    if (!x0 || !w || !out || (ksize != 1 && ksize != 3)) return FGDM_ERR_ARG;
    if (stride == FGDM_STRIDE2_PAD_BR && (ksize != 3 || upsample)) return FGDM_ERR_ARG;
    hipStream_t s = as_stream(stream);
    const int Cin = C0 + C1, taps = ksize * ksize, K = taps * Cin;
    if (B <= 0 || H <= 0 || W <= 0 || Cout <= 0 || C0 <= 0 || C1 < 0) return FGDM_ERR_ARG;
    if (Cin & 63) {
        if (ksize != 3 || C1 || x1 || upsample || (stride != 1 && stride != 2)) return FGDM_ERR_ARG;
        return op_conv3_im2col((const half_t*)x0, C0, w, bias, rowvec, (const half_t*)resid, B, H, W, Cout, stride, act, scale, out, s);
    }
    std::vector<int> kmap(K);
    for (int tap = 0; tap < taps; ++tap)
        for (int c = 0; c < Cin; ++c) kmap[taps == 9 ? ((c >> 6) * 9 + tap) * 64 + (c & 63) : c] = c * taps + tap;
    TmpDev tmp;
    IgemmArgs a{};
    const int prc = op_pack(a, tmp, w, bias, Cout, K, K, false, kmap.data());
    if (prc != FGDM_OK) return prc;
    a.A0 = (const half_t*)x0; a.C0 = C0; a.A1 = (const half_t*)x1; a.C1 = C1;
    a.zero = g_zero_page();
// ... 225 lines not shown
    LoopStep a{};
    a.io = StepIO{x, e_cond, e_uncond, x_out, xin_a, xin_b, log_x, cfg_scale, (size_t)n};
    a.noise = noise; a.mask = mask; a.x0 = x0; a.qnoise = q_noise; a.log_p0 = log_pred_x0;
    a.a_t = a_t; a.a_prev = a_prev; a.sigma = sigma_t; a.s1m = sqrt_one_minus_at;
    a.sa_next = sqrt_ac_next; a.s1m_next = sqrt_one_minus_ac_next; a.mode = LOOP_PLAIN;
    return loop_step(a, as_stream(stream));
}

int fgdm_op_plms_loop_step(const float* x, const float* e_cond, const float* e_uncond, float cfg_scale, int mode, int order,
                           const float* e1, const float* e2, const float* e3, float* e_out, float a_t, float a_prev,
                           float sqrt_one_minus_at, const float* mask, const float* x0, const float* q_noise, float sqrt_ac_next,
                           float sqrt_one_minus_ac_next, float* x_out, float* xin_a, float* xin_b, float* log_x, float* log_pred_x0,
                           int64_t n, void* stream) {
    if (n <= 0 || (e_cond && mode == LOOP_PLAIN)) return FGDM_ERR_ARG;
    LoopStep a{};
    a.io = StepIO{x, e_cond, e_uncond, x_out, xin_a, xin_b, log_x, cfg_scale, (size_t)n};
    a.e1 = e1; a.e2 = e2; a.e3 = e3; a.mask = mask; a.x0 = x0; a.qnoise = q_noise; a.e_out = e_out; a.log_p0 = log_pred_x0;
    a.a_t = a_t; a.a_prev = a_prev; a.s1m = sqrt_one_minus_at; a.sa_next = sqrt_ac_next;
    a.s1m_next = sqrt_one_minus_ac_next; a.mode = mode; a.order = order;
    return loop_step(a, as_stream(stream));
}

int fgdm_op_dpmpp_loop_step(const float* x, const float* e_cond, const float* e_uncond, float cfg_scale, float inv_alpha,
                            float neg_sigma_over_alpha, const float* m1, int update_kind, float c1, float cm0, float cm1,
                            float* m0_out, float* x_out, float* xin_a, float* xin_b, int64_t n, void* stream) {
    if (n <= 0) return FGDM_ERR_ARG;
    DpmppLoopStep a{};
    a.io = StepIO{x, e_cond, e_uncond, x_out, xin_a, xin_b, nullptr, cfg_scale, (size_t)n};
    a.m1 = m1; a.m0_out = m0_out; a.inv_alpha = inv_alpha; a.neg_sigma_over_alpha = neg_sigma_over_alpha; a.c1 = c1; a.cm0 = cm0; a.cm1 = cm1;
    a.kind = update_kind;
    return dpmpp_loop_step(a, as_stream(stream));
}

int fgdm_op_dpm_program_step(const float* x_eval, const float* e_cond, const float* e_uncond, float cfg_scale, float conv_x, float conv_e,
                             float* base, float* hist0, float* hist1, float* hist2, int slot, int nterms, const int32_t* planes,
                             const float* coefs, float* x_out, float* xin_a, float* xin_b, int64_t n, void* stream) {
    if (n <= 0) return FGDM_ERR_ARG;
    DpmProgramStep a{};
    float* const pl[4] = {base, hist0, hist1, hist2};
    if (dpm_program_terms(a, pl, slot, nterms, planes, coefs) != FGDM_OK) return FGDM_ERR_ARG;
    a.io = StepIO{x_eval, e_cond, e_uncond, x_out, xin_a, xin_b, nullptr, cfg_scale, (size_t)n};
    a.conv_x = conv_x; a.conv_e = conv_e;
    return dpm_program_step(a, as_stream(stream));
}

int fgdm_op_ancestral_loop_step(const float* x, const float* eps, float sqrt_recip_ac, float sqrt_recipm1_ac, float coef1, float coef2,
                                float std, const float* noise, const float* mask, const float* x0, const float* q_noise,
                                float sqrt_ac_t, float sqrt_one_minus_ac_t, float* x_out, float* xin, float* log_x, int64_t n,
                                void* stream) {
    if (n <= 0) return FGDM_ERR_ARG;
    AncestralLoopStep a{};
    a.io = StepIO{x, eps, nullptr, x_out, xin, nullptr, log_x, 0.f, (size_t)n};
    a.noise = noise; a.mask = mask; a.x0 = x0; a.qnoise = q_noise;
    a.cr = sqrt_recip_ac; a.crm1 = sqrt_recipm1_ac; a.c1 = coef1; a.c2 = coef2; a.std = std;
    a.sa_t = sqrt_ac_t; a.s1m_t = sqrt_one_minus_ac_t;
    return ancestral_loop_step(a, as_stream(stream));
}

int fgdm_op_invert_loop_step(const float* x, const float* e_cond, const float* e_uncond, float cfg_scale, float cx, float ce,
                             float* x_out, float* xin_a, float* xin_b, float* log_x, int64_t n, void* stream) {
    if (n <= 0) return FGDM_ERR_ARG;
    InvertLoopStep a{};
    a.io = StepIO{x, e_cond, e_uncond, x_out, xin_a, xin_b, log_x, cfg_scale, (size_t)n};
    a.cx = cx; a.ce = ce;
    return invert_loop_step(a, as_stream(stream));
}

int fgdm_replay_plan(int n_walks, const int32_t* lens, const uint64_t* key, const uint32_t* grid_x, const uint64_t* shape, int group_max,
                     int chunk, int32_t* out, int out_cap, int* limits) {
    if (limits) { limits[0] = REPLAY_LOOK; limits[1] = FGDM_MAX_GROUP; }
    if (n_walks < 0 || group_max < 1 || out_cap < 0 || (n_walks && !lens) || (out_cap && !out)) return FGDM_ERR_ARG;
    std::vector<PlanWalk> walks(n_walks);
    size_t u = 0;
    for (int w = 0; w < n_walks; ++w) {
        if (lens[w] < 0 || (lens[w] && (!key || !grid_x || !shape))) return FGDM_ERR_ARG;
        for (int i = 0; i < lens[w]; ++i, ++u) walks[w].push_back(PlanUnit{key[u], grid_x[u], shape[u]});
    }
    std::vector<int32_t> steps;
    replay_plan_chunked(walks.data(), n_walks, chunk, group_max, REPLAY_LOOK, steps);
    for (size_t i = 0; i < steps.size() && i < (size_t)out_cap; ++i) out[i] = steps[i];
    return (int)steps.size();
}

}
```

fgdm_amd/engine.py:

```python
import ctypes as C
import os
from collections import OrderedDict

import numpy as np
import torch

from . import _lib

SD_V1 = dict(in_channels=4, out_channels=4, model_channels=320, attention_resolutions=(4, 2, 1),
             num_res_blocks=2, channel_mult=(1, 2, 4, 4), num_heads=8, context_dim=768)


SD_VAE = dict(ch=128, out_ch=3, ch_mult=(1, 2, 4, 4), num_res_blocks=2, attn_resolutions=(), z_channels=4)


SD_CLIP = dict(vocab_size=49408, hidden_size=768, intermediate_size=3072, num_hidden_layers=12,
               num_attention_heads=12, max_position_embeddings=77)


def make_config(cfg=None, use_adapter=False, n_controlnets=0, hint_channels=3, workspace_bytes=0, vae=None, clip=None,
                num_prompts=1, vae_encoder=False):
    if vae_encoder and not vae:
        raise ValueError('vae_encoder needs the first-stage config: pass vae=True or a ddconfig dict')
    if cfg is not None and ('target' in cfg or any(k not in SD_V1 for k in cfg)):
# ... 260 lines not shown
            v = value.detach()
            if v.dtype not in (torch.float32, torch.float16):
                v = v.float()
            v = v.contiguous()
            dtype = 0 if v.dtype == torch.float32 else 1
            shape = tuple(v.shape)
            ptr = C.c_void_p(v.data_ptr())
            keep = v
        else:
            a = np.ascontiguousarray(value)
            if a.dtype not in (np.float32, np.float16):
                a = a.astype(np.float32)
            dtype = 0 if a.dtype == np.float32 else 1
            shape = a.shape
            ptr = a.ctypes.data_as(C.c_void_p)
            keep = a
        sh = (C.c_int64 * len(shape))(*shape)
        rc = self.lib.fgdm_load_tensor(self.h, key.encode(), ptr, dtype, sh, len(shape))
        del keep
        self._check(rc, f'fgdm_load_tensor({key})')

    def load_state_dict(self, sd, strict=True):
        want = self.param_shapes()
        missing = [k for k in want if k not in sd]
        if strict and missing:
            raise KeyError(f'{len(missing)} parameters missing, e.g. {missing[:3]}')
        for k in want:
            if k in sd:
                self.load_tensor(k, sd[k])
        return missing

    def finalize(self):
        self._check(self.lib.fgdm_finalize_weights(self.h), 'fgdm_finalize_weights')
        self._ctx_policy = ContextCachePolicy()
        self._hint_keys = [None] * self.n_controlnets
        self._conds_key, self._conds_keep = None, None

    def set_hint(self, cn, hint):
        key = (id(hint), hint.data_ptr(), hint._version, tuple(hint.shape))
        if self._hint_keys[cn] is not None and self._hint_keys[cn][0] == key:
            return
        dev = hint.to(self.device, torch.float32).contiguous()
        B, _, Hh, Wh = dev.shape
        self._check(self.lib.fgdm_set_hint(self.h, cn, _ptr(dev), B, Hh, Wh, _stream()), 'fgdm_set_hint')
        self._hint_keys[cn] = (key, hint)

    def set_adapter_conds(self, conds):
        if not conds:
            if self._conds_key is not None:
                self._check(self.lib.fgdm_set_adapter_conds(self.h, None, 0, 0, 0, 0, _stream()), 'fgdm_set_adapter_conds')
                self._conds_key, self._conds_keep = None, None
            return
        key = tuple((id(c), c._version, tuple(c.shape)) for c in conds)
        if key == self._conds_key:
            return
        dev = [c.to(self.device, torch.float32).contiguous() for c in conds]
        B, _, H, W = dev[0].shape
        ptrs = (C.c_void_p * len(dev))(*[c.data_ptr() for c in dev])
        self._check(self.lib.fgdm_set_adapter_conds(self.h, ptrs, len(dev), B, H, W, _stream()), 'fgdm_set_adapter_conds')
        self._conds_key, self._conds_keep = key, list(conds)

    def set_concat(self, c_concat):
        if c_concat is None:
            self._check(self.lib.fgdm_set_concat(self.h, None, 0, 0, 0, 0, _stream()), 'fgdm_set_concat')
            self._concat_key = None
            return
        key = (id(c_concat), c_concat.data_ptr(), c_concat._version, tuple(c_concat.shape))
        if self._concat_key is not None and self._concat_key[0] == key:
            return
        self._concat_key = None
        dev = c_concat.to(self.device, torch.float32).contiguous()
        B, Cc, H, W = dev.shape
        self._check(self.lib.fgdm_set_concat(self.h, _ptr(dev), B, Cc, H, W, _stream()), 'fgdm_set_concat')
        self._concat_key = (key, c_concat)
        self.concat_uploads += 1

    def set_context_tokens(self, tokens):
        tokens = int(tokens)
        if tokens != self._ctx_tokens:
            self._check(self.lib.fgdm_set_context_tokens(self.h, tokens), 'fgdm_set_context_tokens')
            self._ctx_tokens = tokens
            self._ctx_policy = ContextCachePolicy()

    def apply_model(self, x, t, ctx, control_scales=None, flags=0, pcond=None, out=None):
        x = x.to(self.device, torch.float32).contiguous()
        t_int = t_flt = None
        if t.is_floating_point():
            t_flt = t.to(self.device, torch.float32).contiguous()
        else:
            t_int = t.to(self.device, torch.int64).contiguous()
        B, Cc, H, W = x.shape
        if Cc != 4 or ctx.shape[0] != B or t.shape[0] != B:
            raise ValueError(f'apply_model: x {tuple(x.shape)}, t {tuple(t.shape)}, context {tuple(ctx.shape)} do not agree')
        self.set_context_tokens(ctx.shape[1])
        ctx_arg = None
        if self.cache_context and ctx.is_cuda and ctx.dtype == torch.float32 and ctx.is_contiguous():
            verdict = self._ctx_policy.see(ctx)
            if verdict == 'register':
                self._check(self.lib.fgdm_set_context(self.h, _ptr(ctx), B, _stream()), 'fgdm_set_context')
            elif verdict == 'bypass':
                ctx_arg = ctx
        else:
            ctx_arg = ctx.to(self.device, torch.float32).contiguous()
        eps = torch.empty_like(x) if out is None else out
        sc = None
        if control_scales is not None:
            sc = torch.as_tensor(control_scales, dtype=torch.float32).flatten()
            assert sc.numel() == 13 * self.n_controlnets
            sc_host = sc.numpy().copy()
            sc_ptr = sc_host.ctypes.data_as(C.c_void_p)
        else:
            sc_ptr = C.c_void_p(0)
        if pcond is not None:
            if tuple(pcond.shape) != tuple(x.shape):
                raise ValueError(f'pcond / control shape {tuple(pcond.shape)} must equal the latent batch {tuple(x.shape)}')
            pcond = pcond.to(self.device, torch.float32).contiguous()
        rc = self.lib.fgdm_apply_model(self.h, _ptr(x), _ptr(t_int), _ptr(t_flt), _ptr(ctx_arg), _ptr(pcond), sc_ptr, B, H, W,
                                       flags, _ptr(eps), _stream())
        self._check(rc, 'fgdm_apply_model')
        self.pair_calls += bool(flags & _lib.FLAG_CFG_PAIRS)
        return eps

    def clip_encode(self, ids, clip_skip=0):
        ids = torch.as_tensor(ids).to(self.device, torch.int64).contiguous()
        B, T = ids.shape
        out = torch.empty(B, T, self.config.clip_width, device=self.device, dtype=torch.float32)
        self._check(self.lib.fgdm_clip_encode_skip(self.h, _ptr(ids), B, T, int(clip_skip), _ptr(out), _stream()),
                    'fgdm_clip_encode_skip')
        return out

    def vae_decode(self, z, scale=1.0):
        z = z.to(self.device, torch.float32).contiguous()
        B, Cc, H, W = z.shape
        assert Cc == 4
        f = 1 << (self.config.vae_n_levels - 1)
        img = torch.empty(B, self.config.vae_out_ch, H * f, W * f, device=self.device, dtype=torch.float32)
        rc = self.lib.fgdm_vae_decode(self.h, _ptr(z), B, H, W, float(scale), _ptr(img), _stream())
        self._check(rc, 'fgdm_vae_decode')
        return img

    def vae_decode_patches(self, z, scale, ks, stride, f, w_pix, w_tie, max_crops_per_pass=0):
        z = z.to(self.device, torch.float32).contiguous()
        B, Cc, H, W = z.shape
        assert Cc == 4
        w_pix, w_tie = _weights(w_pix, w_tie, self.device, (H, W, ks, stride, int(f)))
        img = torch.empty(B, self.config.vae_out_ch, H * f, W * f, device=self.device, dtype=torch.float32)
        rc = self.lib.fgdm_vae_decode_patches(self.h, _ptr(z), B, H, W, float(scale), ks[0], ks[1], stride[0], stride[1], int(f),
                                              _ptr(w_pix), _ptr(w_tie), int(max_crops_per_pass), _ptr(img), _stream())
        self._check(rc, 'fgdm_vae_decode_patches')
        return img

    def apply_model_patches(self, x, t, ctx, ks, stride, w_pix, w_tie, max_crops_per_pass=0, flags=0):
        x = x.to(self.device, torch.float32).contiguous()
        t_int = t_flt = None
        if t.is_floating_point():
            t_flt = t.to(self.device, torch.float32).contiguous()
        else:
            t_int = t.to(self.device, torch.int64).contiguous()
        B, Cc, H, W = x.shape
        if Cc != 4 or ctx.shape[0] != B or t.shape[0] != B:
            raise ValueError(f'apply_model_patches: x {tuple(x.shape)}, t {tuple(t.shape)}, context {tuple(ctx.shape)} do not agree')
        self.set_context_tokens(ctx.shape[1])
        ctx = ctx.to(self.device, torch.float32).contiguous()
        w_pix, w_tie = _weights(w_pix, w_tie, self.device, (H, W, ks, stride, 1))
        eps = torch.empty_like(x)
        rc = self.lib.fgdm_apply_model_patches(self.h, _ptr(x), _ptr(t_int), _ptr(t_flt), _ptr(ctx), B, H, W, ks[0], ks[1],
                                               stride[0], stride[1], _ptr(w_pix), _ptr(w_tie), int(max_crops_per_pass),
                                               int(flags), _ptr(eps), _stream())
        self._check(rc, 'fgdm_apply_model_patches')
        return eps

    def unfold(self, x, ks, stride, l0=0, n=None, out=None):
        return unfold(x.to(self.device), ks, stride, l0, n, out)

    def fold_weighted(self, crops, w_pix, w_tie, size, stride, crops_per_pass=0, out=None):
        return fold_weighted(crops.to(self.device), w_pix, w_tie, size, stride, crops_per_pass, out)

    def vae_encode(self, image):
        image = image.to(self.device, torch.float32).contiguous()
        B, Cc, H, W = image.shape
        if Cc != 3:
            raise ValueError(f'vae_encode: image {tuple(image.shape)} must have 3 channels')
        f = 1 << (self.config.vae_n_levels - 1)
        moments = torch.empty(B, 2 * self.config.vae_z_channels, H // f, W // f, device=self.device, dtype=torch.float32)
        rc = self.lib.fgdm_vae_encode(self.h, _ptr(image), B, H, W, _ptr(moments), _stream())
        self._check(rc, 'fgdm_vae_encode')
        return moments

    def posterior_sample(self, moments, noise=None, scale=1.0):
        return posterior_sample(moments.to(self.device), None if noise is None else noise.to(self.device), scale)

    def run_block(self, prefix, x, emb=None, ctx=None, x_skip=None):
        f32 = lambda v: None if v is None else v.to(self.device, torch.float32).contiguous()
        x, emb, ctx, x_skip = f32(x), f32(emb), f32(ctx), f32(x_skip)
        if ctx is not None:
            self.set_context_tokens(ctx.shape[1])
        B, Cc, H, W = x.shape
        cap = 4 * B * 1280 * 4 * H * W
        out = torch.empty(cap, device=self.device, dtype=torch.float32)
        n = C.c_int64(0)
        rc = self.lib.fgdm_run_block(self.h, prefix.encode(), _ptr(x), Cc, _ptr(x_skip), 0 if x_skip is None else x_skip.shape[1],
# ... 337 lines not shown
```

fgdm_amd/models.py:

```python
import contextlib

import numpy as np
import torch

from . import _lib, config as _cfg, hack as _hack, patches as _patches, schedule
from . import engine as _k


def _randn(shape, device):
    return torch.randn(shape, device=device)


def plan_noise_segments(steps, step_bytes, max_bytes):
    per = max(1, int(max_bytes) // max(1, int(step_bytes)))
    return [(a, min(a + per, steps)) for a in range(0, steps, per)]


class _Buffers:

    def _register_schedule(self, device, **kw):
        tabs = schedule.ddpm_tables(**kw)
        for k, v in tabs.items():
            setattr(self, k, torch.from_numpy(v).to(device))
        self._host = tabs
        self.num_timesteps = int(tabs['betas'].shape[0])


class DiagonalGaussianDistribution:

    def __init__(self, parameters, deterministic=False):
        self.parameters = parameters
        self.mean, logvar = torch.chunk(parameters, 2, dim=1)
        self.logvar = torch.clamp(logvar, -30.0, 20.0)
        self.deterministic = deterministic
        if deterministic:
            self.var = self.std = torch.zeros_like(self.mean)
        else:
            self.std = torch.exp(0.5 * self.logvar)
            self.var = torch.exp(self.logvar)

    def sample(self, scale=1.0):
        noise = torch.randn(self.mean.shape).to(device=self.parameters.device)
        if self.parameters.is_cuda and not self.deterministic:
            return _k.posterior_sample(self.parameters, noise, scale)
        x = self.mean + self.std * noise
        return x if scale == 1.0 else scale * x

    def mode(self, scale=1.0):
        if self.parameters.is_cuda:
            return _k.posterior_sample(self.parameters, None, scale)
        return self.mean if scale == 1.0 else scale * self.mean

    def kl(self, other=None):
        if self.deterministic:
            return torch.Tensor([0.])
        if other is None:
            return 0.5 * torch.sum(self.mean ** 2 + self.var - 1.0 - self.logvar, dim=[1, 2, 3])
        return 0.5 * torch.sum((self.mean - other.mean) ** 2 / other.var + self.var / other.var - 1.0 - self.logvar + other.logvar,
                               dim=[1, 2, 3])

    def nll(self, sample, dims=(1, 2, 3)):
        if self.deterministic:
            return torch.Tensor([0.])
        return 0.5 * torch.sum(float(np.log(2.0 * np.pi)) + self.logvar + (sample - self.mean) ** 2 / self.var, dim=list(dims))


class DiffusionWrapper:

    def __init__(self, engine, conditioning_key):
        self.diffusion_model = engine
        self.conditioning_key = conditioning_key


_REFUSED_KEYS = {
    'concat': "conditioning_key='concat' hands the UNet cat([x] + c_concat, 1) WITHOUT a context (ddpm.py:1832-1834): the engine "
              "builds UNets whose SpatialTransformers take a text context; use 'hybrid' (c_concat and c_crossattn)",
    'adm': "conditioning_key='adm' hands the UNet class embeddings, y=c_crossattn[0] (ddpm.py:1842-1844): the engine has no "
           'label embedding (num_classes is fixed to None)',
    None: 'conditioning_key=None is the unconditional UNet (ddpm.py:1830-1831): the engine builds UNets whose SpatialTransformers '
          'take a text context',
}


class LatentDiffusion(_Buffers):
    def __init__(self, unet_config=None, engine=None, use_adapter=None, n_controlnets=0, num_prompts=1, timesteps=1000,
                 beta_schedule='linear', linear_start=0.00085, linear_end=0.012, cosine_s=8e-3, given_betas=None,
                 v_posterior=0.0, parameterization='eps', conditioning_key='crossattn', scale_factor=0.18215,
                 channels=4, image_size=32, log_every_t=200, clip_denoised=False, device=0, first_stage_config=None,
                 cond_stage_config=None, first_stage_encoder=False, device_loop=False, **ignored):
        if parameterization != 'eps':
            raise NotImplementedError(f'parameterization={parameterization!r}: only eps-parameterization is implemented (the shipped '
                                      f'configs, models/config.yaml; {_cfg.SD2_LIMIT}; v-prediction checkpoints are refused)')
        if conditioning_key not in ('crossattn', 'hybrid'):
# ... 208 lines not shown
        raise NotImplementedError(f"encoder_posterior of type '{type(encoder_posterior)}' not yet implemented")

    def _context(self, cond):
        if isinstance(cond, dict):
            cc = cond['c_crossattn']
        elif isinstance(cond, (list, tuple)):
            cc = list(cond)
        else:
            cc = [cond]
        if len(cc) == 1:
            return cc[0]
        key = tuple((id(t), t._version) for t in cc)
        memo = getattr(self, '_ctx_cat_memo', None)
        if memo is None or memo[0] != key:
            self._ctx_cat_memo = memo = (key, list(cc), torch.cat(cc, 1))
        return memo[2]

    def _apply_model_patches(self, x_noisy, t, cond, return_ids, sp):
        ncond = len(cond) if isinstance(cond, dict) else 1
        assert ncond == 1
        assert not return_ids
        if getattr(self, 'cond_stage_key', None) in _patches.SPATIAL_COND_KEYS:
            raise NotImplementedError(f"split_input_params with cond_stage_key '{self.cond_stage_key}' (a conditioning that is cut "
                                      'into crops, or crop coordinates) is not supported: only the text branch is')
        if getattr(self.engine, 'n_controlnets', 0):
            raise NotImplementedError('split_input_params: ControlLDM.apply_model has no patch branch in the reference')
        (kh, kw), stride, Ly, Lx = _patches.plan(x_noisy.shape[2], x_noisy.shape[3], sp['ks'], sp['stride'], clamp=False)
        w_pix, w_tie = self._patch_tables(kh, kw, Ly, Lx, sp)
        return self.engine.apply_model_patches(x_noisy, t, self._context(cond), (kh, kw), stride, w_pix, w_tie,
                                               getattr(self, 'max_crops_per_pass', 0))

    def _concat(self, x_noisy, cond):
        if not isinstance(cond, dict):
            raise TypeError("conditioning_key='hybrid' needs a dict cond {'c_concat': [...], 'c_crossattn': [...]} (the reference "
                            f'fails on [x] + None, ddpm.py:1840); got {type(cond).__name__}')
        parts = cond.get('c_concat')
        if not isinstance(parts, (list, tuple)) or not parts or 'c_crossattn' not in cond:
            raise TypeError("conditioning_key='hybrid' needs cond['c_concat'] (a list of tensors) and cond['c_crossattn']")
        if len(parts) == 1:
            cc = parts[0]
        else:
            key = tuple((id(p), p._version) for p in parts)
            memo = getattr(self, '_concat_cat_memo', None)
            if memo is None or memo[0] != key:
                self._concat_cat_memo = memo = (key, list(parts), torch.cat(list(parts), 1))
            cc = memo[2]
        B = x_noisy.shape[0]
        if cc.dim() != 4 or tuple(cc.shape[2:]) != tuple(x_noisy.shape[2:]) or not (cc.shape[0] == B or 2 * cc.shape[0] == B):
            raise ValueError(f'c_concat {tuple(cc.shape)} does not fit the latent batch {tuple(x_noisy.shape)}')
        return cc, (2 * cc.shape[0] == B or self._halves_equal(cc))

    def capture_attention(self, blocks=None, tokens=None, rows='cond', mode='sum', latent=None, **kw):
        if blocks is not None:
            blocks = [blocks] if isinstance(blocks, (str, int)) or (isinstance(blocks, tuple) and isinstance(blocks[0], str)) else list(blocks)
            blocks = [str(b) if isinstance(b, int) and not isinstance(b, bool) else b for b in blocks]
        return self.engine.capture_attention(blocks=blocks, tokens=tokens, rows=rows, mode=mode,
                                             latent=self.image_size if latent is None else latent, **kw)

    def apply_model(self, x_noisy, t, cond, return_ids=False, **kwargs):
        sp = getattr(self, 'split_input_params', None)
        hybrid = self.model.conditioning_key == 'hybrid'
        if hybrid and sp is not None:
            raise NotImplementedError("split_input_params with conditioning_key='hybrid': the reference's patch branch crops c_concat "
                                      'only for its spatial cond_stage_keys (ddpm.py:1061-1071), which are not supported')
        if sp is not None:
            return self._apply_model_patches(x_noisy, t, cond, return_ids, sp)
        if return_ids:
            raise NotImplementedError('return_ids / return_conds needs a model with two outputs; no shipped model has one')
        if hybrid:
            cc, may_pair = self._concat(x_noisy, cond)
            self.engine.set_concat(cc)
            flags = _lib.FLAG_NO_CONTROL | (_lib.FLAG_USE_ORIGINAL if kwargs.get('use_original', False) else 0)
            if kwargs.get('cfg_pairs', False) and may_pair:
                flags |= _lib.FLAG_CFG_PAIRS
            return self.engine.apply_model(x_noisy, t, self._context(cond), flags=flags)
        flags = _lib.FLAG_NO_CONTROL
        if kwargs.get('use_original', False):
            flags |= _lib.FLAG_USE_ORIGINAL
        if 'conds' in kwargs or getattr(self.engine, '_conds_key', None) is not None:
            self.engine.set_adapter_conds(kwargs.get('conds'))
        pcond = kwargs.get('pcond', kwargs.get('control'))
        if kwargs.get('cfg_pairs', False) and (pcond is None or self._halves_equal(pcond)):
            flags |= _lib.FLAG_CFG_PAIRS
        return self.engine.apply_model(x_noisy, t, self._context(cond), flags=flags, pcond=pcond)

    def _halves_equal(self, v):
        key = (id(v), v._version, tuple(v.shape))
        memo = getattr(self, '_halves_memo', None)
        if memo is None or memo[0] != key:
            n = v.shape[0]
            eq = n % 2 == 0 and bool(torch.equal(v[:n // 2], v[n // 2:]))
            self._halves_memo = memo = (key, v, eq)
        return memo[2]

    def _at(self, name, t):
        return [float(v) for v in self._host[name][np.asarray(t.detach().cpu())]]

    def q_sample(self, x_start, t, noise=None):
        noise = torch.randn_like(x_start) if noise is None else noise
        a, b = self._at('sqrt_alphas_cumprod', t), self._at('sqrt_one_minus_alphas_cumprod', t)
        if len(set(a)) == 1:
            return _k.axpby(x_start.contiguous(), a[0], noise.contiguous(), b[0])
        return torch.cat([_k.axpby(x_start[i:i + 1].contiguous(), a[i], noise[i:i + 1].contiguous(), b[i])
                          for i in range(x_start.shape[0])])

    def predict_start_from_noise(self, x_t, t, noise):
        a, b = self._at('sqrt_recip_alphas_cumprod', t), self._at('sqrt_recipm1_alphas_cumprod', t)
        assert len(set(a)) == 1, 'per-sample timesteps: call per sample'
        return _k.axpby(x_t.contiguous(), a[0], noise.contiguous(), -b[0])

    def p_sample(self, x, c, t, clip_denoised=False, repeat_noise=False, return_x0=False, temperature=1.,
                 noise_dropout=0., noise=None, **kwargs):
        if clip_denoised or noise_dropout > 0.:
            raise NotImplementedError('clip_denoised / noise_dropout are not used by the latent configs')
        ti = int(t[0])
        assert bool((t == ti).all()), 'p_sample expects one timestep per call'
        eps = self.apply_model(x, t, c, **kwargs)
        h = self._host
        if noise is None:
            noise = _randn((1, *x.shape[1:]) if repeat_noise else x.shape, x.device)
            noise = noise.expand_as(x).contiguous()
        std = 0.0 if ti == 0 else float(np.exp(0.5 * h['posterior_log_variance_clipped'][ti])) * temperature
        out = _k.ancestral_step(x.contiguous(), eps, h['sqrt_recip_alphas_cumprod'][ti],
                                h['sqrt_recipm1_alphas_cumprod'][ti], h['posterior_mean_coef1'][ti],
                                h['posterior_mean_coef2'][ti], std, noise if ti != 0 else None)
        if return_x0:
            return out, self.predict_start_from_noise(x, t, eps)
        return out

    def _ancestral_plan(self, cond, img, timesteps, mask, x0, host_hooks, kwargs):
        from . import samplers
        eng = self.engine
        if not getattr(self, 'device_loop', False) or host_hooks or timesteps < 1 or not hasattr(eng, 'sample_ancestral'):
            return None
        if set(kwargs) - {'repeat_noise', 'temperature'} or self.clip_denoised:
            return None
        if getattr(self, 'split_input_params', None) is not None or img.dim() != 4 or img.shape[1] != 4:
            return None
        if mask is not None and (x0 is None or tuple(x0.shape) != tuple(img.shape)):
            return None
        if not isinstance(self, ControlLDM):
            if isinstance(cond, dict) and cond.get('c_concat') is None:
                cond = cond.get('c_crossattn')
            if isinstance(cond, (list, tuple)) and len(cond) == 1:
                cond = cond[0]
        return samplers._loop_cond(self, cond, None, False)

    def _device_ancestral(self, plan, img, timesteps, mask, x0, log_every_t, repeat_noise=False, temperature=1.):
        ctx, _, flags, control_scales = plan
        h = self._host
        ts = list(reversed(range(timesteps)))
        tab = lambda name: [float(h[name][t]) for t in ts]
        tables = {k: tab(k) for k in ('sqrt_recip_alphas_cumprod', 'sqrt_recipm1_alphas_cumprod', 'posterior_mean_coef1',
                                      'posterior_mean_coef2')}
        tables['std'] = [0.0 if t == 0 else float(np.exp(0.5 * h['posterior_log_variance_clipped'][t])) * temperature for t in ts]
        m = None
        if mask is not None:
            m = mask.to(img.dtype).expand_as(img).contiguous()
            tables['sqrt_alphas_cumprod_t'] = tab('sqrt_alphas_cumprod')
            tables['sqrt_one_minus_alphas_cumprod_t'] = tab('sqrt_one_minus_alphas_cumprod')
        logs = [j for j, t in enumerate(ts) if log_every_t and (t % log_every_t == 0 or t == timesteps - 1)]
        inter = []
        step_bytes = img.numel() * 4 * (1 if mask is None else 2)
        for a, b in plan_noise_segments(len(ts), step_bytes, getattr(self, 'max_loop_noise_bytes', 256 << 20)):
            sn = torch.empty(b - a, *img.shape, device=img.device, dtype=torch.float32)
            qn = None if mask is None else torch.empty_like(sn)
            for k in range(b - a):
# ... 23 lines not shown
            timesteps = min(timesteps, start_T)
        if mask is not None:
            assert x0 is not None and x0.shape[2:3] == mask.shape[2:3]
        plan = self._ancestral_plan(cond, img, timesteps, mask, x0, bool(callback or img_callback), kwargs)
        if plan is not None:
            img, logged = self._device_ancestral(plan, img, timesteps, mask, x0, log_every_t if return_intermediates else None, **kwargs)
            return (img, inter + logged) if return_intermediates else img
        for i in reversed(range(0, timesteps)):
            ts = torch.full((b,), i, device=self.device, dtype=torch.long)
            img = self.p_sample(img, cond, ts, clip_denoised=self.clip_denoised, **kwargs)
            if mask is not None:
                img_orig = self.q_sample(x0, ts)
                img = _k.mask_blend(img_orig.contiguous(), img.contiguous(),
                                    mask.to(img.dtype).expand_as(img).contiguous())
            if i % log_every_t == 0 or i == timesteps - 1:
                inter.append(img)
            if callback:
                callback(i)
            if img_callback:
                img_callback(img, i)
        return (img, inter) if return_intermediates else img

    def sample(self, cond, batch_size=16, return_intermediates=False, x_T=None, verbose=True, timesteps=None,
               quantize_denoised=False, mask=None, x0=None, shape=None, **kwargs):
        if shape is None:
            shape = (batch_size, self.channels, self.image_size, self.image_size)
        if cond is not None:
            if isinstance(cond, dict):
                cond = {k: (v[:batch_size] if not isinstance(v, list) else [u[:batch_size] for u in v])
                        for k, v in cond.items()}
            else:
                cond = [c[:batch_size] for c in cond] if isinstance(cond, list) else cond[:batch_size]
        return self.p_sample_loop(cond, shape, return_intermediates=return_intermediates, x_T=x_T, verbose=verbose,
                                  timesteps=timesteps, quantize_denoised=quantize_denoised, mask=mask, x0=x0, **kwargs)


class ControlLDM(LatentDiffusion):

    def __init__(self, unet_config=None, n_controlnets=1, only_mid_control=False, control_key='hint',
                 control_stage_config=None, **kw):
        kw.setdefault('use_adapter', False)
        kw.setdefault('image_size', 64)
        self._check_control_stage(unet_config, control_stage_config)
        super().__init__(unet_config=unet_config, n_controlnets=n_controlnets, **kw)
        self.control_key = control_key
        self.only_mid_control = only_mid_control
        self.n_controlnets = n_controlnets
        self.control_scales = [1.0] * 13

    @staticmethod
    def _check_control_stage(unet_config, control_stage_config):
        if control_stage_config is None:
            return
        ckind, ccfg, cflags = _cfg.unet_params(control_stage_config)
        _, ucfg, _ = _cfg.unet_params(unet_config)
        ucfg = dict(_k.SD_V1 if ucfg is None else ucfg)
        sd2 = _cfg._SD2_KEYS
        diff = [k for k in list(ccfg) + [k for k in sd2 if k not in ccfg] if k != 'out_channels' and
                tuple(np.atleast_1d(ccfg.get(k, sd2.get(k)))) != tuple(np.atleast_1d(ucfg.get(k, sd2.get(k))))]
        if ckind not in (None, 'controlnet') or diff or cflags.get('hint_channels', 3) != 3:
            raise NotImplementedError(f'control_stage_config must be a ControlNet matching unet_config (differs in {diff})')

    @classmethod
    def engine_args(cls, unet_config=None, n_controlnets=1, control_stage_config=None, **kw):
        kw.setdefault('use_adapter', False)
        cls._check_control_stage(unet_config, control_stage_config)
        return super().engine_args(unet_config=unet_config, n_controlnets=n_controlnets, **kw)

    def _scales(self):
        sc = list(self.control_scales)
        if len(sc) == 13:
            sc = sc * self.n_controlnets
        assert len(sc) == 13 * self.n_controlnets, 'control_scales: 13 per control model'
        return sc

    def apply_model(self, x_noisy, t, cond, *args, **kwargs):
        assert isinstance(cond, dict)
        ctx = self._context(cond)
        hints = cond.get('c_concat')
        flags = _lib.FLAG_ONLY_MID_CONTROL if self.only_mid_control else 0
        if kwargs.get('cfg_pairs', False):
            flags |= _lib.FLAG_CFG_PAIRS
        if hints is None:
            return self.engine.apply_model(x_noisy, t, ctx, flags=flags | _lib.FLAG_NO_CONTROL)
        if self.n_controlnets == 1:
            hints = [hints[0] if len(hints) == 1 else torch.cat(hints, 1)]
        assert len(hints) == self.n_controlnets
        for k, h in enumerate(hints):
            self.engine.set_hint(k, h)
        return self.engine.apply_model(x_noisy, t, ctx, control_scales=self._scales(), flags=flags)

    def get_unconditional_conditioning(self, N):
        return self.get_learned_conditioning([""] * N)
```

fgdm_amd/samplers.py:

```python
import numpy as np
import torch

from . import engine as _k
from . import schedule


def _randn(shape, device):
    return torch.randn(shape, device=device)


def _loop_cond(m, c, uc, cfg_on, sampler=None):
    from . import _lib, models
    pair = _lib.FLAG_CFG_PAIRS if cfg_on else 0
    if isinstance(m, models.ControlLDM):
        if type(m).apply_model is not models.ControlLDM.apply_model:
            return None
        if cfg_on and not isinstance(sampler, ControlDDIMSampler):
            return None
        if not isinstance(c, dict) or len(c.get('c_crossattn') or ()) != 1 or not torch.is_tensor(c['c_crossattn'][0]):
            return None
        if cfg_on and (not isinstance(uc, dict) or sampler._cat_cond(uc, c) is None):
            return None
        hints = c.get('c_concat')
        flags = pair | (_lib.FLAG_ONLY_MID_CONTROL if m.only_mid_control else 0)
# ... 5 lines not shown
        if len(hints) != m.n_controlnets:
            return None
        for k, h in enumerate(hints):
            m.engine.set_hint(k, h)
        return ctx, uctx, flags, m._scales()
    if type(m).apply_model is not models.LatentDiffusion.apply_model or m.model.conditioning_key != 'crossattn':
        return None
    if not torch.is_tensor(c) or getattr(m.engine, '_conds_key', None) is not None:
        return None
    if cfg_on and (not torch.is_tensor(uc) or tuple(uc.shape) != tuple(c.shape)):
        return None
    return c, uc if cfg_on else None, _lib.FLAG_NO_CONTROL | pair, None


def _loop_plan(m, sampler, cond, uc, scales, mask, x0, img, host_hooks, kwargs, entry='sample_ddim_ex'):
    eng = getattr(m, 'engine', None)
    if (sampler is not None and not getattr(sampler, 'device_loop', False)) or eng is None or not hasattr(eng, entry) or host_hooks or kwargs:
        return None
    if getattr(m, 'split_input_params', None) is not None or getattr(sampler, '_dyn', None) is not None:
        return None
    if getattr(m, 'parameterization', 'eps') != 'eps' or not hasattr(m, '_host') or img.dim() != 4 or img.shape[1] != 4:
        return None
    on = [uc is not None and s != 1. for s in scales]
    if any(on) != all(on):
        return None
    if mask is not None and (x0 is None or tuple(x0.shape) != tuple(img.shape)):
        return None
    return _loop_cond(m, cond, uc, all(on), sampler)


class _SamplerBase:
    def __init__(self, model, schedule="linear", **kwargs):
        self.model = model
        self.ddpm_num_timesteps = model.num_timesteps
        self.schedule = schedule

    def register_buffer(self, name, attr):
        if isinstance(attr, torch.Tensor) and attr.device != torch.device(self.model.device):
            attr = attr.to(self.model.device)
        setattr(self, name, attr)

    def make_schedule(self, ddim_num_steps, ddim_discretize="uniform", ddim_eta=0., verbose=True):
        self.ddim_timesteps = schedule.ddim_timesteps(ddim_discretize, ddim_num_steps, self.ddpm_num_timesteps)
        if verbose:
            print(f'Selected timesteps for ddim sampler: {self.ddim_timesteps}')
        ac = self.model.alphas_cumprod
        assert ac.shape[0] == self.ddpm_num_timesteps, 'alphas have to be defined for each timestep'
        f32 = lambda v: torch.as_tensor(v).clone().detach().to(torch.float32).to(self.model.device)
        ac_h = ac.detach().float().cpu()
        self.register_buffer('betas', f32(self.model.betas))
        self.register_buffer('alphas_cumprod', f32(ac))
        self.register_buffer('alphas_cumprod_prev', f32(self.model.alphas_cumprod_prev))
        self.register_buffer('sqrt_alphas_cumprod', f32(torch.sqrt(ac_h)))
        self.register_buffer('sqrt_one_minus_alphas_cumprod', f32(torch.sqrt(1. - ac_h)))
        self.register_buffer('log_one_minus_alphas_cumprod', f32(torch.log(1. - ac_h)))
        self.register_buffer('sqrt_recip_alphas_cumprod', f32(torch.sqrt(1. / ac_h)))
        self.register_buffer('sqrt_recipm1_alphas_cumprod', f32(torch.sqrt(1. / ac_h - 1)))
        sig, a, ap, s1m = schedule.ddim_tables(ac_h.numpy(), self.ddim_timesteps, ddim_eta)
        if verbose:
            print(f'Selected alphas for ddim sampler: a_t: {a}; a_(t-1): {ap}')
            print(f'For the chosen value of eta, which is {ddim_eta}, this results in the following sigma_t '
                  f'schedule for ddim sampler {sig}')
        self.ddim_sigmas, self.ddim_alphas, self.ddim_alphas_prev, self.ddim_sqrt_one_minus_alphas = sig, a, ap, s1m
        acp_h = self.model.alphas_cumprod_prev.detach().float().cpu()
        self.register_buffer('ddim_sigmas_for_original_num_steps',
                             ddim_eta * torch.sqrt((1 - acp_h) / (1 - ac_h) * (1 - ac_h / acp_h)))

    def _tables(self, use_original_steps):
        if not use_original_steps:
            return self.ddim_alphas, self.ddim_alphas_prev, self.ddim_sqrt_one_minus_alphas, self.ddim_sigmas
        h = lambda v: v.detach().float().cpu().numpy()
        return (h(self.model.alphas_cumprod), h(self.model.alphas_cumprod_prev),
                h(self.model.sqrt_one_minus_alphas_cumprod), h(self.ddim_sigmas_for_original_num_steps))

    @staticmethod
    def _batch_of(conditioning):
        if isinstance(conditioning, dict):
            v = conditioning[list(conditioning.keys())[0]]
            while isinstance(v, (list, tuple)):
                v = v[0]
            return v.shape[0]
        return conditioning.shape[0]

    def _eval_pair(self, x, t, c, uc, scale, **kwargs):
        if uc is None or scale == 1.:
            return self.model.apply_model(x, t, c, **kwargs), None
        x_in, t_in = torch.cat([x] * 2), torch.cat([t] * 2)
        c_in = self._batched_cond(uc, c)
        if c_in is None:
            return self.model.apply_model(x, t, c, **kwargs), self.model.apply_model(x, t, uc, **kwargs)
        if getattr(self.model, 'engine', None) is not None:
            kwargs = dict(kwargs, cfg_pairs=True)
        e_u, e_c = self.model.apply_model(x_in, t_in, c_in, **kwargs).chunk(2)
        return e_c.contiguous(), e_u.contiguous()

    @staticmethod
    def _cat_cond(uc, c):
        return torch.cat([uc, c])

    @staticmethod
    def _leaves(c, out):
        if torch.is_tensor(c):
            out.append(c)
        elif isinstance(c, dict):
            for k in sorted(c):
                _SamplerBase._leaves(c[k], out)
        elif isinstance(c, (list, tuple)):
            for v in c:
                _SamplerBase._leaves(v, out)
        return out

    def _batched_cond(self, uc, c):
        leaves = self._leaves(uc, []) + self._leaves(c, [])
        key = tuple((id(t), t._version) for t in leaves)
        memo = getattr(self, '_cin_memo', None)
        if memo is not None and memo[0] == key:
            return memo[2]
        c_in = self._cat_cond(uc, c)
        self._cin_memo = (key, leaves, c_in)
        return c_in

    def _x_prev(self, x, e_cond, e_uncond, scale, index, tabs, temperature, noise_dropout, repeat_noise,
                want_pred_x0=True):
        alphas, alphas_prev, s1m, sigmas = tabs
        sigma = float(sigmas[index])
        shape = (1, *x.shape[1:]) if repeat_noise else x.shape
        noise = _randn(shape, x.device)
        if sigma == 0.0:
            noise = None
        else:
            if repeat_noise:
                noise = noise.expand_as(x).contiguous()
            if temperature != 1.:
                noise = noise * temperature
            if noise_dropout > 0.:
                noise = torch.nn.functional.dropout(noise, p=noise_dropout)
        return _k.ddim_step(x.contiguous(), e_cond, e_uncond, scale, float(alphas[index]), float(alphas_prev[index]),
                            sigma, float(s1m[index]), noise, want_pred_x0)

    def _blend_mask(self, img, mask, x0, ts):
        img_orig = self.model.q_sample(x0, ts)
        m = mask.to(img.dtype).expand_as(img).contiguous()
        return _k.mask_blend(img_orig.contiguous(), img.contiguous(), m)

    def stochastic_encode(self, x0, t, use_original_steps=False, noise=None):
        if use_original_steps:
            sa, s1m = self.sqrt_alphas_cumprod.cpu().numpy(), self.sqrt_one_minus_alphas_cumprod.cpu().numpy()
        else:
            sa, s1m = np.sqrt(self.ddim_alphas), self.ddim_sqrt_one_minus_alphas
        noise = torch.randn_like(x0) if noise is None else noise
        ti = np.asarray(t.detach().cpu())
        assert (ti == ti.flat[0]).all(), 'one encode index per call'
        return _k.axpby(x0.contiguous(), float(sa[ti.flat[0]]), noise.contiguous(), float(s1m[ti.flat[0]]))


    def _mask_kw(self, mask, x0, qn, img, timesteps):
        if mask is None:
            return {}
        h = self.model._host
        return dict(mask=mask.to(img.dtype).expand_as(img).contiguous(), x0=x0, q_noise=torch.stack(qn),
                    sqrt_alphas_cumprod_t=[h['sqrt_alphas_cumprod'][int(t)] for t in timesteps],
                    sqrt_one_minus_alphas_cumprod_t=[h['sqrt_one_minus_alphas_cumprod'][int(t)] for t in timesteps])

    @staticmethod
    def _log_steps(total_steps, log_every_t):
        return [i for i in range(total_steps) if (total_steps - i - 1) % log_every_t == 0 or i == 0]


class DDIMSampler(_SamplerBase):
    def __init__(self, model, schedule="linear", device_loop=False, **kwargs):
        super().__init__(model, schedule, **kwargs)
        self.device_loop = bool(device_loop)

    def _device_loop(self, plan, img, timesteps, tabs, scales, mask, x0, temperature, log_steps):
        ctx, uctx, flags, control_scales = plan
        S = len(timesteps)
        alphas, alphas_prev, s1m, sigmas = (np.asarray(t)[:S] for t in tabs)
        qn, sn = [], []
        for i in range(S):
            if mask is not None:
                qn.append(torch.randn_like(x0))
            noise = _randn(img.shape, img.device)
            if float(sigmas[S - 1 - i]) != 0.0 and temperature != 1.:
                noise = noise * temperature
            if sigmas.any():
                sn.append(noise)
        kw = self._mask_kw(mask, x0, qn, img, timesteps)
        cfg_on = uctx is not None
        return self.model.engine.sample_ddim_ex(img, ctx, uctx, scales[0] if cfg_on else 1.0, [int(t) for t in timesteps], alphas,
                                                alphas_prev, s1m, sigmas=sigmas, cfg_scales=scales if cfg_on else None,
                                                step_noise=torch.stack(sn) if sn else None, log_steps=log_steps,
                                                control_scales=control_scales, flags=flags, **kw)

    def sample(self, S, batch_size, shape, conditioning=None, callback=None, normals_sequence=None,
               img_callback=None, quantize_x0=False, eta=0., mask=None, x0=None, temperature=1., noise_dropout=0.,
               score_corrector=None, corrector_kwargs=None, verbose=True, x_T=None, log_every_t=100,
               unconditional_guidance_scale=1., unconditional_conditioning=None, inference_loss=False, **kwargs):
        if conditioning is not None:
            cbs = self._batch_of(conditioning)
            if cbs != batch_size:
                print(f"Warning: Got {cbs} conditionings but batch-size is {batch_size}")
        self.make_schedule(ddim_num_steps=S, ddim_eta=eta, verbose=verbose)
        C, H, W = shape
        size = (batch_size, C, H, W)
        if verbose:
            print(f'Data shape for DDIM sampling is {size}, eta {eta}')
        return self.ddim_sampling(conditioning, size, callback=callback, img_callback=img_callback,
                                  quantize_denoised=quantize_x0, mask=mask, x0=x0, ddim_use_original_steps=False,
                                  noise_dropout=noise_dropout, temperature=temperature,
                                  score_corrector=score_corrector, corrector_kwargs=corrector_kwargs, x_T=x_T,
                                  log_every_t=log_every_t, unconditional_guidance_scale=unconditional_guidance_scale,
                                  unconditional_conditioning=unconditional_conditioning,
                                  inference_loss=inference_loss, **kwargs)

    def ddim_sampling(self, cond, shape, x_T=None, ddim_use_original_steps=False, callback=None, timesteps=None,
                      quantize_denoised=False, mask=None, x0=None, img_callback=None, log_every_t=100,
                      temperature=1., noise_dropout=0., score_corrector=None, corrector_kwargs=None,
                      unconditional_guidance_scale=1., unconditional_conditioning=None, inference_loss=False,
                      **kwargs):
        device = self.model.betas.device
        b = shape[0]
        img = _randn(shape, device) if x_T is None else x_T.to(device, torch.float32)
        if timesteps is None:
            timesteps = self.ddpm_num_timesteps if ddim_use_original_steps else self.ddim_timesteps
        elif not ddim_use_original_steps:
            n = self.ddim_timesteps.shape[0]
            timesteps = self.ddim_timesteps[:int(min(timesteps / n, 1) * n) - 1]
        intermediates = {'x_inter': [img], 'pred_x0': [img]}
        time_range = list(reversed(range(0, timesteps))) if ddim_use_original_steps else np.flip(timesteps)
        total_steps = timesteps if ddim_use_original_steps else timesteps.shape[0]
        ucg = getattr(self, '_ucg', None)
        scales = [unconditional_guidance_scale if ucg is None else ucg[i] for i in range(total_steps)] \
            if ucg is None or len(ucg) >= total_steps else None
        hooks = bool(callback or img_callback or score_corrector is not None or noise_dropout > 0. or quantize_denoised
                     or inference_loss)
        plan = None if scales is None or total_steps < 1 else \
            _loop_plan(self.model, self, cond, unconditional_conditioning, scales, mask, x0, img, hooks, kwargs)
        if plan is not None:
            log_steps = self._log_steps(total_steps, log_every_t)
            img, x_inter, pred = self._device_loop(plan, img, list(reversed([int(t) for t in time_range])),
                                                   self._tables(ddim_use_original_steps), scales, mask, x0, temperature, log_steps)
            intermediates['x_inter'] += list(x_inter)
            intermediates['pred_x0'] += list(pred)
            return img, intermediates
        for i, step in enumerate(time_range):
            index = total_steps - i - 1
            ts = torch.full((b,), int(step), device=device, dtype=torch.long)
            if mask is not None:
                assert x0 is not None
                img = self._blend_mask(img, mask, x0, ts)
            img, pred_x0 = self.p_sample_ddim(img, cond, ts, index=index, use_original_steps=ddim_use_original_steps,
                                              quantize_denoised=quantize_denoised, temperature=temperature,
                                              noise_dropout=noise_dropout, score_corrector=score_corrector,
                                              corrector_kwargs=corrector_kwargs,
                                              unconditional_guidance_scale=unconditional_guidance_scale,
                                              unconditional_conditioning=unconditional_conditioning, i=i,
                                              inference_loss=inference_loss, **kwargs)
            if callback:
                callback(i)
            if img_callback:
                img_callback(pred_x0, i)
            if index % log_every_t == 0 or index == total_steps - 1:
                intermediates['x_inter'].append(img)
                intermediates['pred_x0'].append(pred_x0)
        return img, intermediates

    def p_sample_ddim(self, x, c, t, index, repeat_noise=False, use_original_steps=False, quantize_denoised=False,
                      temperature=1., noise_dropout=0., score_corrector=None, corrector_kwargs=None,
                      unconditional_guidance_scale=1., unconditional_conditioning=None, i=0, inference_loss=False,
                      **kwargs):
        if inference_loss or kwargs.get('return_conds'):
            raise NotImplementedError('attention-alignment guidance / joint condition update need a model with a '
                                      'tuple output; no shipped model provides one (dead code in the reference)')
        if quantize_denoised:
            raise NotImplementedError('quantize_denoised needs a VQ first stage (not part of the latent-diffusion path)')
        uc, scale = unconditional_conditioning, unconditional_guidance_scale
        e_u = None
        if uc is None or scale == 1.:
            e_c = self.model.apply_model(x, t, c, **kwargs)
        elif 'composable_diffusion' in kwargs:
            kw = {k: v for k, v in kwargs.items() if k != 'composable_diffusion'}
            n = kwargs['composable_diffusion'] + 1
            out = self.model.apply_model(torch.cat([x] * n), torch.cat([t] * n), torch.cat([uc, c]), **kw)
            e_c = _k.axpby(out[:1].contiguous(), float(2 - n), None, 0.0)
            for k in range(1, n):
                e_c = _k.axpby(e_c, 1.0, out[k:k + 1].contiguous(), 1.0)
        elif 'augmented_conditoning' in kwargs:
            kw = {k: v for k, v in kwargs.items() if k not in ('augmented_conditoning', 'ac')}
            e_un, e_t, e_ac = self.model.apply_model(torch.cat([x] * 3), torch.cat([t] * 3),
                                                     torch.cat([uc, c, kwargs['ac']]), **kw).chunk(3)
            e_c = _k.cfg_combine(e_t.contiguous(), e_ac.contiguous(), scale)
            e_u = e_un.contiguous()
        else:
            e_c, e_u = self._eval_pair(x, t, c, uc, scale, **kwargs)
        if score_corrector is not None:
            assert self.model.parameterization == "eps"
            e_c = _k.cfg_combine(e_c, e_u, scale) if e_u is not None else e_c
            e_c, e_u = score_corrector.modify_score(self.model, e_c, x, t, c, **(corrector_kwargs or {})), None
        return self._x_prev(x, e_c, e_u, scale, index, self._tables(use_original_steps), temperature,
                            noise_dropout, repeat_noise)

    def decode(self, x_latent, cond, t_start, unconditional_guidance_scale=1.0, unconditional_conditioning=None,
               use_original_steps=False, callback=None):
        timesteps = np.arange(self.ddpm_num_timesteps) if use_original_steps else self.ddim_timesteps
        timesteps = timesteps[:t_start]
        total_steps = timesteps.shape[0]
        x_dec = x_latent
        plan = None if total_steps < 1 or getattr(self, '_ucg', None) is not None else \
            _loop_plan(self.model, self, cond, unconditional_conditioning, [unconditional_guidance_scale] * total_steps, None, None, x_latent,
                            bool(callback), {})
        if plan is not None:
            return self._device_loop(plan, x_latent, [int(t) for t in timesteps], self._tables(use_original_steps),
                                     [unconditional_guidance_scale] * total_steps, None, None, 1., ())[0]
        for i, step in enumerate(np.flip(timesteps)):
            index = total_steps - i - 1
            ts = torch.full((x_latent.shape[0],), int(step), device=x_latent.device, dtype=torch.long)
            x_dec, _ = self.p_sample_ddim(x_dec, cond, ts, index=index, use_original_steps=use_original_steps,
                                          unconditional_guidance_scale=unconditional_guidance_scale,
                                          unconditional_conditioning=unconditional_conditioning)
            if callback:
                callback(i)
        return x_dec


class PLMSSampler(_SamplerBase):
    def __init__(self, model, schedule="linear", device_loop=False, **kwargs):
        super().__init__(model, schedule, **kwargs)
        self.device_loop = bool(device_loop)

    def _device_loop(self, plan, img, timesteps, tabs, scale, mask, x0, log_steps):
        ctx, uctx, flags, control_scales = plan
        S = len(timesteps)
        alphas, alphas_prev, s1m = (np.asarray(t)[:S] for t in tabs[:3])
        qn = []
        for i in range(S):
            if mask is not None:
                qn.append(torch.randn_like(x0))
            for _ in range(2 if i == 0 else 1):
                _randn(img.shape, img.device)
        kw = self._mask_kw(mask, x0, qn, img, timesteps)
        return self.model.engine.sample_plms(img, ctx, uctx, scale if uctx is not None else 1.0, [int(t) for t in timesteps],
                                             alphas, alphas_prev, s1m, log_steps=log_steps, control_scales=control_scales,
                                             flags=flags, **kw)

    def make_schedule(self, ddim_num_steps, ddim_discretize="uniform", ddim_eta=0., verbose=True):
        if ddim_eta != 0:
            raise ValueError('ddim_eta must be 0 for PLMS')
        super().make_schedule(ddim_num_steps, ddim_discretize, ddim_eta, verbose)

    def sample(self, S, batch_size, shape, conditioning=None, callback=None, normals_sequence=None,
               img_callback=None, quantize_x0=False, eta=0., mask=None, x0=None, temperature=1., noise_dropout=0.,
               score_corrector=None, corrector_kwargs=None, verbose=True, x_T=None, log_every_t=100,
               unconditional_guidance_scale=1., unconditional_conditioning=None, **kwargs):
        if conditioning is not None:
            cbs = self._batch_of(conditioning)
            if cbs != batch_size:
                print(f"Warning: Got {cbs} conditionings but batch-size is {batch_size}")
        self.make_schedule(ddim_num_steps=S, ddim_eta=eta, verbose=verbose)
        C, H, W = shape
        size = (batch_size, C, H, W)
        if verbose:
            print(f'Data shape for PLMS sampling is {size}')
# ... 365 lines not shown
```

include/fgdm.h:

```cpp
#ifndef FGDM_H
#define FGDM_H
#include <stdint.h>
#ifdef __cplusplus
extern "C" {
#endif

#define FGDM_MAX_LEVELS 8
#define FGDM_MAX_CONTROLNETS 4

typedef struct fgdm_engine fgdm_engine;

typedef struct fgdm_config {
    int32_t in_channels, out_channels, model_channels, num_res_blocks;
    int32_t n_levels;
    int32_t channel_mult[FGDM_MAX_LEVELS];
    int32_t n_attention_resolutions;
    int32_t attention_resolutions[FGDM_MAX_LEVELS];
    int32_t num_heads, context_dim;
    int32_t use_adapter;
    int32_t n_controlnets;
    int32_t hint_channels;
    int64_t workspace_bytes;
    int32_t vae_ch, vae_n_levels;
    int32_t vae_ch_mult[FGDM_MAX_LEVELS];
    int32_t vae_num_res_blocks, vae_z_channels, vae_out_ch;
    int32_t clip_layers, clip_width, clip_heads, clip_mlp, clip_vocab, clip_max_len;
    int32_t n_extra_adapters;
    int32_t vae_encoder;
    int32_t reserved0;
    int32_t num_head_channels;
    int32_t use_linear_in_transformer;
} fgdm_config;

#define FGDM_DTYPE_F32 0
#define FGDM_DTYPE_F16 1

#define FGDM_FLAG_USE_ORIGINAL 1
#define FGDM_FLAG_ONLY_MID_CONTROL 2
#define FGDM_FLAG_NO_CONTROL 4
#define FGDM_FLAG_CFG_PAIRS 8

int fgdm_create(const fgdm_config* cfg, int device, fgdm_engine** out);
void fgdm_destroy(fgdm_engine* e);
const char* fgdm_last_error(const fgdm_engine* e);

int fgdm_param_count(const fgdm_config* cfg);
int fgdm_param_info(const fgdm_config* cfg, int index, char* name, int name_cap, int64_t* shape, int* ndim);

int fgdm_load_tensor(fgdm_engine* e, const char* key, const void* data, int dtype, const int64_t* shape, int ndim);
int fgdm_finalize_weights(fgdm_engine* e);

int fgdm_set_hint(fgdm_engine* e, int cn, const float* hint, int B, int Hh, int Wh, void* stream);

int fgdm_set_adapter_conds(fgdm_engine* e, const float* const* conds, int n_conds, int B, int H, int W, void* stream);

int fgdm_set_context(fgdm_engine* e, const float* ctx, int B, void* stream);
int fgdm_set_context_tokens(fgdm_engine* e, int tokens);
int fgdm_get_context_tokens(const fgdm_engine* e);
#define FGDM_ATTENTION_CAPTURE_MAX_KEYS 256
#define FGDM_CAPTURE_ROWS_ALL 0
#define FGDM_CAPTURE_ROWS_COND 1
#define FGDM_CAPTURE_ROWS_UNCOND 2
#define FGDM_CAPTURE_SUM 0
#define FGDM_CAPTURE_LAST 1
#define FGDM_ATTENTION_CAPTURE_SIZE_V1 48
typedef struct fgdm_attention_capture {
    int64_t struct_size;
    const int32_t* tokens;
    uint32_t block_mask;
    int32_t n_tokens;
    int32_t rows;
    int32_t mode;
    int32_t batch, latent_h, latent_w;
    int32_t reserved0;
} fgdm_attention_capture;
int fgdm_attention_capture_set(fgdm_engine* e, const fgdm_attention_capture* plan);
int fgdm_attention_capture_reset(fgdm_engine* e, void* stream);
int fgdm_attention_capture_info(fgdm_engine* e, int block, int64_t shape[3], int32_t* n_evals);
int fgdm_attention_capture_block_size(fgdm_engine* e, int block, int32_t* h, int32_t* w);
int fgdm_attention_capture_read(fgdm_engine* e, int block, float* dst_device, void* stream);

int fgdm_set_concat(fgdm_engine* e, const float* c_concat, int B, int Cc, int H, int W, void* stream);
int fgdm_apply_model(fgdm_engine* e, const float* x, const int64_t* t, const float* t_float, const float* ctx,
                     const float* pcond, const float* control_scales, int B, int H, int W, int flags, float* eps_out,
                     void* stream);

int fgdm_clip_encode(fgdm_engine* e, const int64_t* ids, int B, int T, float* out, void* stream);
int fgdm_clip_encode_skip(fgdm_engine* e, const int64_t* ids, int B, int T, int clip_skip, float* out, void* stream);

int fgdm_vae_decode(fgdm_engine* e, const float* z, int B, int H, int W, float scale, float* image, void* stream);
int fgdm_vae_encode(fgdm_engine* e, const float* image, int B, int H, int W, float* moments, void* stream);
int fgdm_posterior_sample(const float* moments, const float* noise , float scale, float* z,
                          int B, int zc, int HW, void* stream);

int fgdm_unfold(const float* x, int B, int C, int H, int W, int kh, int kw, int sh, int sw, int l0, int n, float* crops,
                void* stream);
int fgdm_fold_weighted(const float* crops, const float* w_pix, const float* w_tie, int B, int C, int Ho, int Wo, int kh, int kw,
                       int sh, int sw, int crops_per_pass, float* out, void* stream);
int fgdm_vae_decode_patches(fgdm_engine* e, const float* z, int B, int H, int W, float scale, int kh, int kw, int sh, int sw,
                            int f, const float* w_pix, const float* w_tie, int max_crops_per_pass, float* image, void* stream);
int fgdm_apply_model_patches(fgdm_engine* e, const float* x, const int64_t* t, const float* t_float, const float* ctx, int B,
                             int H, int W, int kh, int kw, int sh, int sw, const float* w_pix, const float* w_tie,
                             int max_crops_per_pass, int flags, float* eps_out, void* stream);

int fgdm_image_to_uint8(const float* image, int B, int C, int H, int W, int mode, uint8_t* out, void* stream);
int fgdm_resize_linear_uint8(const uint8_t* src, int B, int H, int W, int C, int Ho, int Wo, uint8_t* dst, void* stream);
int fgdm_uint8_to_hint(const uint8_t* src, int B, int H, int W, int C, float* hint, void* stream);

int fgdm_controlnet(fgdm_engine* e, int cn, const float* x, const int64_t* t, const float* ctx, int B, int H, int W,
                    float* out, int64_t out_capacity_floats, void* stream);

int fgdm_run_block(fgdm_engine* e, const char* prefix, const float* x, int C, const float* x_skip, int Cs, const float* emb,
                   const float* ctx, int B, int H, int W, float* out, int64_t out_capacity_floats, int64_t* out_numel,
                   void* stream);

int fgdm_ddim_step(const float* x, const float* e_cond, const float* e_uncond, float cfg_scale, float a_t,
                   float a_prev, float sigma_t, float sqrt_one_minus_at, const float* noise, float* x_prev,
                   float* pred_x0, float* e_out, int64_t n, void* stream);
int fgdm_plms_combine(const float* e_t, const float* e1, const float* e2, const float* e3, int order,
                      float* e_prime, int64_t n, void* stream);
int fgdm_axpby(const float* a, float ca, const float* b, float cb, float* y, int64_t n, void* stream);
int fgdm_mask_blend(const float* a, const float* b, const float* mask, float* y, int64_t n, void* stream);
int fgdm_ancestral_step(const float* x, const float* eps, float sqrt_recip_ac, float sqrt_recipm1_ac, float coef1,
                        float coef2, float std, const float* noise, float* out, int64_t n, void* stream);

int fgdm_sample_ddim(fgdm_engine* e, float* x, const float* cond, const float* uncond, float cfg_scale, int S,
                     const int64_t* timesteps, const float* alphas, const float* alphas_prev,
                     const float* sqrt_one_minus_alphas, const float* control_scales, int B, int H, int W,
                     int flags, void* stream);

#define FGDM_DDIM_PARAMS_SIZE_V1 192
typedef struct fgdm_ddim_params {
    int64_t struct_size;
    float* x;
    const float* cond;
    const float* uncond;
    const int64_t* timesteps;
    const float* alphas;
    const float* alphas_prev;
    const float* sqrt_one_minus_alphas;
    const float* control_scales;
    const float* sigmas;
    const float* cfg_scales;
    const float* step_noise;
    const float* mask;
    const float* x0;
    const float* q_noise;
    const float* sqrt_alphas_cumprod_t;
    const float* sqrt_one_minus_alphas_cumprod_t;
    const int32_t* log_steps;
    float* x_inter_out;
    float* pred_x0_out;
    float cfg_scale;
    int32_t S;
    int32_t B;
    int32_t H;
    int32_t W;
    int32_t flags;
    int32_t n_log;
    int32_t reserved0;
} fgdm_ddim_params;
int fgdm_sample_ddim_ex(fgdm_engine* e, const fgdm_ddim_params* p, void* stream);

#define FGDM_PLMS_PARAMS_SIZE_V1 168
typedef struct fgdm_plms_params {
    int64_t struct_size;
    float* x;
    const float* cond;
// ... 217 lines not shown
```

Measured before the change: 8.150.

## Precompute timestep-embedding table per sampling schedule and read rows per step

When the sampler announces its DDIM timestep schedule, the engine runs the timestep-embedding MLP chain once for all unique timesteps, for the UNet and every ControlNet, and stores the results in a device table. Each apply_model call with a uniform timestep then points the embedding context at a table row (stride 0 across the batch) instead of launching four kernels per net per step. This removes small per-step launches and GEMMs. It adds API surface, a table allocation and a bookkeeping path that must be invalidated correctly when the schedule or the weights change.

```diff
diff --git a/fgdm_amd/_lib.py b/fgdm_amd/_lib.py
--- a/fgdm_amd/_lib.py
+++ b/fgdm_amd/_lib.py
@@ -109,6 +109,12 @@
     'fgdm_set_adapter_conds': (_i, [_p, _p, _i, _i, _i, _i, _p]),
     'fgdm_set_context': (_i, [_p, _p, _i, _p]),
     'fgdm_apply_model': (_i, [_p, _p, _p, _p, _p, _p, _p, _i, _i, _i, _i, _p, _p]),
+    'fgdm_set_timestep_schedule': (_i, [_p, C.POINTER(_i64), _i, _p]),
+    'fgdm_apply_model_uniform_t': (_i, [_p, _p, _p, _i64, _p, _p, _p, _i, _i, _i, _i, _p, _p]),
+    'fgdm_emb_table_stats': (_i, [_p, C.POINTER(_i64), C.POINTER(_i64), C.POINTER(C.c_int32)]),
+    'fgdm_embed': (_i, [_p, _i, _p, _i, _p, _i64, C.POINTER(C.c_int32), _p]),
+    'fgdm_emb_table_read': (_i, [_p, _i, _p, _i64, C.POINTER(C.c_int32), C.POINTER(C.c_int32), _p]),
+    'fgdm_emb_plan': (_i, [C.POINTER(_i64), _i, C.POINTER(_i64), C.POINTER(C.c_int32), C.POINTER(_i64), _i, C.POINTER(C.c_int32)]),
     'fgdm_clip_encode': (_i, [_p, _p, _i, _i, _p, _p]),
     'fgdm_clip_encode_skip': (_i, [_p, _p, _i, _i, _i, _p, _p]),
     'fgdm_set_context_tokens': (_i, [_p, _i]),
diff --git a/fgdm_amd/csrc/emb_plan.h b/fgdm_amd/csrc/emb_plan.h
--- /dev/null
+++ b/fgdm_amd/csrc/emb_plan.h
@@ -0,0 +1,20 @@
+#pragma once
+#include <cstdint>
+#include <cstring>
+#include <vector>
+
+template <typename T> inline int emb_plan_find(const std::vector<T>& rows, T t) {
+    for (size_t r = 0; r < rows.size(); ++r)
+        if (memcmp(&rows[r], &t, sizeof(T)) == 0) return (int)r;
+    return -1;
+}
+
+template <typename T> inline void emb_plan(const T* t, int S, std::vector<T>& rows, std::vector<int32_t>& row_of) {
+    rows.clear();
+    row_of.assign(S > 0 ? S : 0, -1);
+    for (int k = 0; k < S; ++k) {
+        int r = emb_plan_find(rows, t[k]);
+        if (r < 0) { r = (int)rows.size(); rows.push_back(t[k]); }
+        row_of[k] = r;
+    }
+}
diff --git a/fgdm_amd/csrc/engine.hip b/fgdm_amd/csrc/engine.hip
--- a/fgdm_amd/csrc/engine.hip
+++ b/fgdm_amd/csrc/engine.hip
@@ -1,6 +1,7 @@
 #include "model.h"
 #include "knobs.h"
 #include "replay.h"
+#include "emb_plan.h"
 
 #include <algorithm>
 #include <array>
@@ -206,6 +207,19 @@
     ReplayStats replay_stats;
     struct Deferred { const GemmW* w; Tensor src; int idx; float scale; Arena* owner; };
     Prof prof;
+    struct EmbSchedule {
+        bool valid = false, frac = false;
+        std::vector<int64_t> ti;
+        std::vector<float> tf;
+        std::vector<int32_t> row_of;
+        std::vector<float*> tab;
+        std::vector<size_t> cap;
+        int rows() const { return (int)(frac ? tf.size() : ti.size()); }
+    } emb_sched;
+    bool emb_table_on = true;
+    static constexpr int EMB_TABLE_M = 64;
+    int emb_row = -1;
+    int64_t emb_chain_launches = 0, emb_table_reads = 0;
 
     const ParamSlot* slot(const std::string& name) {
         auto it = params.find(name);
@@ -754,19 +768,73 @@
         return FGDM_OK;
     }
 
-    int embed(Net& n, const int64_t* t, const float* tf, int B, float** emb_all) {
+    int embed_rows(Net& n, const int64_t* t, const float* tf, int B, float* dst) {
         const int mc = cfg.model_channels;
         Tensor te = talloc(1, 1, B, mc), e1, e2;
         if (!te.p) return fail(FGDM_ERR_NOMEM, "workspace");
         if (timestep_embed(t, tf, te.p, B, mc, B, s) != FGDM_OK) return fail(FGDM_ERR_HIP, "timestep_embed");
         { Epi e; e.act = ACT_SILU; e.rps = 1; CHK(linear(n.time0, te, e, &e1)); }
         { Epi e; e.act = ACT_SILU; e.rps = 1; CHK(linear(n.time2, e1, e, &e2)); }
-        *emb_all = (float*)ar->alloc((size_t)B * n.emb_total * sizeof(float));
-        if (!*emb_all) return fail(FGDM_ERR_NOMEM, "workspace");
-        { Epi e; e.out_kind = OUT_F32; e.out = *emb_all; e.ld_out = n.emb_total; e.rps = 1; CHK(linear(n.emb_all, e2, e, nullptr)); }
+        { Epi e; e.out_kind = OUT_F32; e.out = dst; e.ld_out = n.emb_total; e.rps = 1; CHK(linear(n.emb_all, e2, e, nullptr)); }
         tfree(te); tfree(e1); tfree(e2);
-        return FGDM_OK;
-    }
+        emb_chain_launches += 4;
+        return FGDM_OK;
+    }
+    int net_index(const Net& n) const { return &n == &unet ? 0 : 1 + (int)(&n - cns.data()); }
+    int embed(Net& n, const int64_t* t, const float* tf, int B, EmbCtx* ec, float** owned) {
+        *owned = nullptr;
+        if (emb_row >= 0) {
+            *ec = EmbCtx{emb_sched.tab[net_index(n)] + (size_t)emb_row * n.emb_total, 0};
+            ++emb_table_reads;
+            return FGDM_OK;
+        }
+        *owned = (float*)ar->alloc((size_t)B * n.emb_total * sizeof(float));
+        if (!*owned) return fail(FGDM_ERR_NOMEM, "workspace");
+        *ec = EmbCtx{*owned, n.emb_total};
+        return embed_rows(n, t, tf, B, *owned);
+    }
+    int set_emb_schedule(const int64_t* tih, const float* tfh, int S) {
+        EmbSchedule& sc = emb_sched;
+        sc.valid = false;
+        if (!emb_table_on || S <= 0 || (!tih && !tfh)) return FGDM_OK;
+        if (!finalized) return fail(FGDM_ERR_STATE, "weights not finalized");
+        sc.frac = tfh != nullptr;
+        sc.ti.clear(); sc.tf.clear();
+        if (sc.frac) emb_plan(tfh, S, sc.tf, sc.row_of);
+        else emb_plan(tih, S, sc.ti, sc.row_of);
+        const int R = sc.rows();
+        const size_t tbytes = (size_t)R * (sc.frac ? sizeof(float) : sizeof(int64_t));
+        void* tdev = ar->alloc(tbytes);
+        if (!tdev) return fail(FGDM_ERR_NOMEM, "workspace");
+        HIP_TRY(hipMemcpyAsync(tdev, sc.frac ? (const void*)sc.tf.data() : (const void*)sc.ti.data(), tbytes, hipMemcpyHostToDevice, s));
+        HIP_TRY(hipStreamSynchronize(s));
+        sc.tab.resize(1 + cns.size(), nullptr);
+        sc.cap.resize(1 + cns.size(), 0);
+        for (size_t i = 0; i < sc.tab.size(); ++i) {
+            Net& n = i == 0 ? unet : cns[i - 1];
+            const size_t need = (size_t)R * n.emb_total;
+            if (sc.cap[i] < need) {
+                if (sc.tab[i]) (void)hipFree(sc.tab[i]);
+                sc.tab[i] = nullptr; sc.cap[i] = 0;
+                if (hipMalloc(&sc.tab[i], need * sizeof(float)) != hipSuccess) return fail(FGDM_ERR_NOMEM, "hipMalloc (timestep-embedding table)");
+                sc.cap[i] = need;
+            }
+            LayerHints twins(*this, i > 0);
+            for (int r0 = 0; r0 < R; r0 += EMB_TABLE_M) {
+                const int nr = std::min(EMB_TABLE_M, R - r0);
+                CHK(embed_rows(n, sc.frac ? nullptr : (const int64_t*)tdev + r0, sc.frac ? (const float*)tdev + r0 : nullptr, nr,
+                               sc.tab[i] + (size_t)r0 * n.emb_total));
+            }
+        }
+        ar->release(tdev);
+        sc.valid = true;
+        return FGDM_OK;
+    }
+    void drop_emb_schedule() {
+        for (float* p : emb_sched.tab) if (p) (void)hipFree(p);
+        emb_sched = EmbSchedule{};
+    }
+    int emb_row_of(int64_t t) const { return emb_sched.valid && !emb_sched.frac && t >= 0 ? emb_plan_find(emb_sched.ti, t) : -1; }
 
     int adapter_fwd(Net& n, const Tensor& x4, Tensor feats[4]) { return adapter_run(n.ad_conv_in, n.ad_body, x4, feats); }
     int adapter_run(const GemmW& conv_in, const std::vector<AdapterBlk>& body, const Tensor& x4, Tensor feats[4]) {
@@ -993,8 +1061,8 @@
         if (!(n.guided.B == B || 2 * n.guided.B == B) || n.guided.H != x4.H || n.guided.W != x4.W)
             return fail(FGDM_ERR_ARG, "cached hint does not match the batch / latent size");
         float* emb = nullptr;
-        CHK(embed(n, t, tf, B, &emb));
-        EmbCtx ec{emb, n.emb_total};
+        EmbCtx ec{nullptr, 0};
+        CHK(embed(n, t, tf, B, &ec, &emb));
         Tensor h;
         int64_t off = 0;
         auto zero_conv = [&](const GemmW& zw, const Tensor& src, int idx) -> int {
@@ -1042,7 +1110,7 @@
         CHK(block_fwd(n.middle, h, !defer, nullptr, ec, ctx16, nullptr, &m));
         CHK(zero_conv(n.mid_out, m, -1));
         if (!defer) tfree(m);
-        ar->release(emb);
+        if (emb) ar->release(emb);
         return FGDM_OK;
     }
 
@@ -1057,7 +1125,9 @@
     }
 
     int apply_model(const float* x, const int64_t* t, const float* tf, const float* ctx, const float* pcond,
-                    const float* scales, int B, int H, int W, int flags, float* eps_out) {
+                    const float* scales, int B, int H, int W, int flags, float* eps_out, int row = -1) {
+        struct RowScope { int& r; ~RowScope() { r = -1; } } scope{emb_row};
+        emb_row = emb_sched.valid && row < emb_sched.rows() && B <= EMB_TABLE_M ? row : -1;
         if (!cap.on) return apply_model_walk(x, t, tf, ctx, pcond, scales, B, H, W, flags, eps_out);
         if (!finalized) return fail(FGDM_ERR_STATE, "weights not finalized");
         if (B <= 0 || H <= 0 || W <= 0) return fail(FGDM_ERR_ARG, "bad shape");
@@ -1090,8 +1160,8 @@
         } else if (nchw_f32_to_nhwc_f16(x, x4.p, B, 4, HW, 4, s) != FGDM_OK) return fail(FGDM_ERR_HIP, "layout kernel");
         if (ctx && f32_to_f16(ctx, ctx16.p, ctx16.numel(), s) != FGDM_OK) return fail(FGDM_ERR_HIP, "convert kernel");
         float* emb = nullptr;
-        CHK(embed(n, t, tf, B, &emb));
-        EmbCtx ec{emb, n.emb_total};
+        EmbCtx ec{nullptr, 0};
+        CHK(embed(n, t, tf, B, &ec, &emb));
 
         const bool use_adapter = n.has_adapter && !(flags & FGDM_FLAG_USE_ORIGINAL);
         const int Bs = pairs ? B / 2 : B;
@@ -1199,7 +1269,7 @@
         tfree(g);
         tfree(x4);
         if (ctx16.p) tfree(ctx16);
-        ar->release(emb);
+        if (emb) ar->release(emb);
         return FGDM_OK;
     }
 
@@ -1487,8 +1557,8 @@
         if (hist_planes) hist = (float*)e->arena.alloc(hist_planes * n * sizeof(float));
         void* tdev = e->arena.alloc((size_t)K * Bm * (times_int ? sizeof(int64_t) : sizeof(float)));
         if (!tdev || (hist_planes && !hist)) return e->fail(FGDM_ERR_NOMEM, "workspace");
-        if (times_int) return upload_repeated(times_int, K, Bm, t_int = (int64_t*)tdev, s);
-        return upload_repeated(times_float, K, Bm, t_float = (float*)tdev, s);
+        CHK(times_int ? upload_repeated(times_int, K, Bm, t_int = (int64_t*)tdev, s) : upload_repeated(times_float, K, Bm, t_float = (float*)tdev, s));
+        return e->set_emb_schedule(times_int, times_float, K);
     }
     float* plane(int j) const { return hist + (size_t)j * n; }
     int seed() {
@@ -1498,7 +1568,7 @@
     }
     int eval(int k) {
         return e->apply_model(x2, t_int ? t_int + (size_t)k * Bm : nullptr, t_float ? t_float + (size_t)k * Bm : nullptr, nullptr, nullptr,
-                              control_scales, Bm, H, W, flags, eps);
+                              control_scales, Bm, H, W, flags, eps, e->emb_sched.valid ? e->emb_sched.row_of[k] : -1);
     }
     void feed(StepIO& io) const { io.xin_a = x2; io.xin_b = cfg_on ? x2 + n : nullptr; }
     StepIO step_io(int i, float cfg) const {
@@ -1512,6 +1582,7 @@
     int end(int rc) {
         e->arena.release(x2); e->arena.release(eps); e->arena.release(c2); e->arena.release(hist);
         e->arena.release(t_int); e->arena.release(t_float);
+        e->emb_sched.valid = false;
         return rc;
     }
 };
@@ -1552,6 +1623,7 @@
     e->pair_launch = knob_on(KNOB_PAIR_LAUNCH);
     e->group_max = std::max(2, std::min(FGDM_MAX_GROUP, knob_int(KNOB_GROUP_MAX)));
     e->gn_group = knob_on(KNOB_GN_GROUP);
+    e->emb_table_on = knob_on(KNOB_EMB_TABLE);
     if (e->twin_streams && !e->cns.empty()) {
         if (hipStreamCreateWithFlags(&e->s2, hipStreamNonBlocking) != hipSuccess ||
             hipEventCreateWithFlags(&e->ev_fork, hipEventDisableTiming) != hipSuccess ||
@@ -1578,6 +1650,7 @@
     e->drop_concat();
     e->drop_context();
     e->drop_adapter_conds();
+    e->drop_emb_schedule();
     e->capture_free();
     if (knob_text(KNOB_PAIR_DEBUG) && e->replay_stats.replayed)
         fprintf(stderr, "[fgdm] grouped twin launches: %ld of %ld replayed launches were fused (%ld problems)\n", e->replay_stats.fused, e->replay_stats.replayed, e->replay_stats.problems);
@@ -1646,6 +1719,7 @@
     int rc = e->ensure_device();
     if (rc != FGDM_OK) return rc;
     e->drop_context();
+    e->emb_sched.valid = false;
     e->drop_adapter_conds();
     for (auto& n : e->cns) if (n.guided.p) { (void)hipFree(n.guided.p); n.guided = Tensor{}; }
     for (int c = 0; c < (int)e->comps.size(); ++c) { rc = e->repack(c); if (rc != FGDM_OK) return rc; }
@@ -1728,6 +1802,63 @@
                      void* stream) {
     if (!e || !x || (!t && !t_float) || !eps_out) return FGDM_ERR_ARG;
     return scoped_call(e, stream, [&] { return e->apply_model(x, t, t_float, ctx, pcond, control_scales, B, H, W, flags, eps_out); });
+}
+
+int fgdm_set_timestep_schedule(fgdm_engine* e, const int64_t* timesteps, int S, void* stream) {
+    if (!e || S < 0 || (S > 0 && !timesteps)) return FGDM_ERR_ARG;
+    for (int k = 0; k < S; ++k)
+        if (timesteps[k] < 0) return e->fail(FGDM_ERR_ARG, "fgdm_set_timestep_schedule: a timestep is negative");
+    return scoped_call(e, stream, [&] { return e->set_emb_schedule(timesteps, nullptr, S); });
+}
+
+int fgdm_apply_model_uniform_t(fgdm_engine* e, const float* x, const int64_t* t, int64_t t_uniform, const float* ctx,
+                               const float* pcond, const float* control_scales, int B, int H, int W, int flags, float* eps_out,
+                               void* stream) {
+    if (!e || !x || !t || !eps_out) return FGDM_ERR_ARG;
+    return scoped_call(e, stream, [&] {
+        return e->apply_model(x, t, nullptr, ctx, pcond, control_scales, B, H, W, flags, eps_out, e->emb_row_of(t_uniform));
+    });
+}
+
+int fgdm_emb_table_stats(fgdm_engine* e, int64_t* chain_launches, int64_t* table_reads, int32_t* rows) {
+    if (!e || !chain_launches || !table_reads || !rows) return FGDM_ERR_ARG;
+    *chain_launches = e->emb_chain_launches;
+    *table_reads = e->emb_table_reads;
+    *rows = e->emb_sched.valid ? e->emb_sched.rows() : 0;
+    return FGDM_OK;
+}
+
+static Net* emb_net(fgdm_engine* e, int net) {
+    if (net < 0 || net > (int)e->cns.size()) { e->fail(FGDM_ERR_ARG, "no such net"); return nullptr; }
+    return net == 0 ? &e->unet : &e->cns[net - 1];
+}
+int fgdm_embed(fgdm_engine* e, int net, const int64_t* t, int B, float* out, int64_t out_capacity_floats, int32_t* width, void* stream) {
+    if (!e) return FGDM_ERR_ARG;
+    Net* n = emb_net(e, net);
+    if (!n) return FGDM_ERR_ARG;
+    if (width) *width = n->emb_total;
+    if (!out) return FGDM_OK;
+    if (!t || B <= 0) return FGDM_ERR_ARG;
+    if (!e->finalized) return e->fail(FGDM_ERR_STATE, "weights not finalized");
+    if ((int64_t)B * n->emb_total > out_capacity_floats) return e->fail(FGDM_ERR_ARG, "fgdm_embed: output buffer too small");
+    return scoped_call(e, stream, [&] {
+        fgdm_engine::LayerHints twins(*e, net > 0);
+        return e->embed_rows(*n, t, nullptr, B, out);
+    });
+}
+int fgdm_emb_table_read(fgdm_engine* e, int net, float* out, int64_t out_capacity_floats, int32_t* rows, int32_t* width, void* stream) {
+    if (!e || !out) return FGDM_ERR_ARG;
+    Net* n = emb_net(e, net);
+    if (!n) return FGDM_ERR_ARG;
+    if (!e->emb_sched.valid) return e->fail(FGDM_ERR_STATE, "no timestep schedule is announced (fgdm_set_timestep_schedule; FGDM_EMB_TABLE=0?)");
+    const int R = e->emb_sched.rows();
+    if (rows) *rows = R;
+    if (width) *width = n->emb_total;
+    const int64_t cnt = (int64_t)R * n->emb_total;
+    if (cnt > out_capacity_floats) return e->fail(FGDM_ERR_ARG, "fgdm_emb_table_read: output buffer too small");
+    if (hipMemcpyAsync(out, e->emb_sched.tab[net], (size_t)cnt * sizeof(float), hipMemcpyDeviceToDevice, as_stream(stream)) != hipSuccess)
+        return e->fail(FGDM_ERR_HIP, "hipMemcpyAsync (timestep-embedding table)");
+    return FGDM_OK;
 }
 
 int fgdm_set_adapter_conds(fgdm_engine* e, const float* const* conds, int n_conds, int B, int H, int W, void* stream) {
diff --git a/fgdm_amd/csrc/knobs.h b/fgdm_amd/csrc/knobs.h
--- a/fgdm_amd/csrc/knobs.h
+++ b/fgdm_amd/csrc/knobs.h
@@ -34,6 +34,7 @@
     X(PAIR_LAUNCH, "FGDM_PAIR_LAUNCH", "1", "fgdm_create; 0: no grouped launches of twin layers")                               \
     X(GROUP_MAX, "FGDM_GROUP_MAX", FGDM_STR(FGDM_MAX_GROUP), "fgdm_create; problems per grouped launch, clamped to [2, FGDM_MAX_GROUP]") \
     X(GN_GROUP, "FGDM_GN_GROUP", "1", "fgdm_create; 0: single-pass GroupNorm launches stay out of the grouped launches")        \
+    X(EMB_TABLE, "FGDM_EMB_TABLE", "1", "fgdm_create; 0: the timestep-embedding chain runs at every step, no table per sampling")  \
     X(PAIR_DEBUG, "FGDM_PAIR_DEBUG", nullptr, "set (to anything): fgdm_destroy prints how many replayed launches were fused")   \
     X(PROF_DUMP, "FGDM_PROF_DUMP", nullptr, "path: fgdm_profile_end writes the per-shape time table there")                     \
     X(BENCH_DATA_SCALE, "FGDM_BENCH_DATA_SCALE", "1", "atof; scale of the random operands of fgdm_bench_igemm / _attention")
diff --git a/fgdm_amd/csrc/ops_abi.hip b/fgdm_amd/csrc/ops_abi.hip
--- a/fgdm_amd/csrc/ops_abi.hip
+++ b/fgdm_amd/csrc/ops_abi.hip
@@ -1,5 +1,6 @@
 #include "engine_shared.h"
 #include "replay_plan.h"
+#include "emb_plan.h"
 
 static int op_pack(IgemmArgs& a, TmpDev& tmp, const float* w, const float* bias, int N, int K, int Ks, bool geglu,
                    const int* kmap = nullptr, const float* gamma = nullptr, const float* beta = nullptr) {
@@ -391,4 +392,15 @@
     return (int)steps.size();
 }
 
-}
+int fgdm_emb_plan(const int64_t* timesteps, int S, int64_t* rows, int32_t* row_of, const int64_t* probes, int n_probes, int32_t* probe_rows) {
+    if (S < 0 || n_probes < 0 || (S && (!timesteps || !rows || !row_of)) || (n_probes && (!probes || !probe_rows))) return FGDM_ERR_ARG;
+    std::vector<int64_t> r;
+    std::vector<int32_t> of;
+    emb_plan(timesteps, S, r, of);
+    for (size_t i = 0; i < r.size(); ++i) rows[i] = r[i];
+    for (int k = 0; k < S; ++k) row_of[k] = of[k];
+    for (int j = 0; j < n_probes; ++j) probe_rows[j] = emb_plan_find(r, probes[j]);
+    return (int)r.size();
+}
+
+}
diff --git a/fgdm_amd/engine.py b/fgdm_amd/engine.py
--- a/fgdm_amd/engine.py
+++ b/fgdm_amd/engine.py
@@ -366,7 +366,36 @@
             self._ctx_tokens = tokens
             self._ctx_policy = ContextCachePolicy()
 
-    def apply_model(self, x, t, ctx, control_scales=None, flags=0, pcond=None, out=None):
+    def set_timestep_schedule(self, timesteps):
+        ts = [int(v) for v in timesteps] if timesteps is not None else []
+        arr = (C.c_int64 * max(len(ts), 1))(*ts)
+        self._check(self.lib.fgdm_set_timestep_schedule(self.h, arr, len(ts), _stream()), 'fgdm_set_timestep_schedule')
+
+    def emb_table_stats(self):
+        a, b, r = C.c_int64(), C.c_int64(), C.c_int32()
+        self._check(self.lib.fgdm_emb_table_stats(self.h, C.byref(a), C.byref(b), C.byref(r)), 'fgdm_emb_table_stats')
+        return dict(chain_launches=a.value, table_reads=b.value, rows=r.value)
+
+    def embed(self, net, t):
+        t = t.to(self.device, torch.int64).contiguous()
+        out = torch.empty(t.shape[0], self._emb_width(net), device=self.device, dtype=torch.float32)
+        self._check(self.lib.fgdm_embed(self.h, int(net), _ptr(t), t.shape[0], _ptr(out), out.numel(), None, _stream()), 'fgdm_embed')
+        return out
+
+    def _emb_width(self, net):
+        w = C.c_int32()
+        self._check(self.lib.fgdm_embed(self.h, int(net), None, 0, None, 0, C.byref(w), None), 'fgdm_embed')
+        return w.value
+
+    def emb_table(self, net):
+        rows = self.emb_table_stats()['rows']
+        out = torch.empty(max(rows, 1), self._emb_width(net), device=self.device, dtype=torch.float32)
+        r, w = C.c_int32(), C.c_int32()
+        self._check(self.lib.fgdm_emb_table_read(self.h, int(net), _ptr(out), out.numel(), C.byref(r), C.byref(w), _stream()),
+                    'fgdm_emb_table_read')
+        return out[:r.value]
+
+    def apply_model(self, x, t, ctx, control_scales=None, flags=0, pcond=None, out=None, t_uniform=None):
         x = x.to(self.device, torch.float32).contiguous()
         t_int = t_flt = None
         if t.is_floating_point():
@@ -399,8 +428,12 @@
             if tuple(pcond.shape) != tuple(x.shape):
                 raise ValueError(f'pcond / control shape {tuple(pcond.shape)} must equal the latent batch {tuple(x.shape)}')
             pcond = pcond.to(self.device, torch.float32).contiguous()
-        rc = self.lib.fgdm_apply_model(self.h, _ptr(x), _ptr(t_int), _ptr(t_flt), _ptr(ctx_arg), _ptr(pcond), sc_ptr, B, H, W,
-                                       flags, _ptr(eps), _stream())
+        if t_uniform is not None and t_int is not None:
+            rc = self.lib.fgdm_apply_model_uniform_t(self.h, _ptr(x), _ptr(t_int), int(t_uniform), _ptr(ctx_arg), _ptr(pcond), sc_ptr,
+                                                     B, H, W, flags, _ptr(eps), _stream())
+        else:
+            rc = self.lib.fgdm_apply_model(self.h, _ptr(x), _ptr(t_int), _ptr(t_flt), _ptr(ctx_arg), _ptr(pcond), sc_ptr, B, H, W,
+                                           flags, _ptr(eps), _stream())
         self._check(rc, 'fgdm_apply_model')
         self.pair_calls += bool(flags & _lib.FLAG_CFG_PAIRS)
         return eps
diff --git a/fgdm_amd/models.py b/fgdm_amd/models.py
--- a/fgdm_amd/models.py
+++ b/fgdm_amd/models.py
@@ -9,6 +9,11 @@
 
 def _randn(shape, device):
     return torch.randn(shape, device=device)
+
+
+def _t_uniform_kw(kwargs):
+    tu = kwargs.get('t_uniform')
+    return {} if tu is None else {'t_uniform': tu}
 
 
 def plan_noise_segments(steps, step_bytes, max_bytes):
@@ -383,7 +388,7 @@
         pcond = kwargs.get('pcond', kwargs.get('control'))
         if kwargs.get('cfg_pairs', False) and (pcond is None or self._halves_equal(pcond)):
             flags |= _lib.FLAG_CFG_PAIRS
-        return self.engine.apply_model(x_noisy, t, self._context(cond), flags=flags, pcond=pcond)
+        return self.engine.apply_model(x_noisy, t, self._context(cond), flags=flags, pcond=pcond, **_t_uniform_kw(kwargs))
 
     def _halves_equal(self, v):
         key = (id(v), v._version, tuple(v.shape))
@@ -573,13 +578,13 @@
         if kwargs.get('cfg_pairs', False):
             flags |= _lib.FLAG_CFG_PAIRS
         if hints is None:
-            return self.engine.apply_model(x_noisy, t, ctx, flags=flags | _lib.FLAG_NO_CONTROL)
+            return self.engine.apply_model(x_noisy, t, ctx, flags=flags | _lib.FLAG_NO_CONTROL, **_t_uniform_kw(kwargs))
         if self.n_controlnets == 1:
             hints = [hints[0] if len(hints) == 1 else torch.cat(hints, 1)]
         assert len(hints) == self.n_controlnets
         for k, h in enumerate(hints):
             self.engine.set_hint(k, h)
-        return self.engine.apply_model(x_noisy, t, ctx, control_scales=self._scales(), flags=flags)
+        return self.engine.apply_model(x_noisy, t, ctx, control_scales=self._scales(), flags=flags, **_t_uniform_kw(kwargs))
 
     def get_unconditional_conditioning(self, N):
         return self.get_learned_conditioning([""] * N)
diff --git a/fgdm_amd/samplers.py b/fgdm_amd/samplers.py
--- a/fgdm_amd/samplers.py
+++ b/fgdm_amd/samplers.py
@@ -111,7 +111,12 @@
             return v.shape[0]
         return conditioning.shape[0]
 
+    def _t_kw(self, t, kwargs):
+        tu = getattr(self, '_t_uniform', None)
+        return dict(kwargs, t_uniform=tu[1]) if tu is not None and t is tu[0] else kwargs
+
     def _eval_pair(self, x, t, c, uc, scale, **kwargs):
+        kwargs = self._t_kw(t, kwargs)
         if uc is None or scale == 1.:
             return self.model.apply_model(x, t, c, **kwargs), None
         x_in, t_in = torch.cat([x] * 2), torch.cat([t] * 2)
@@ -272,26 +277,33 @@
             intermediates['x_inter'] += list(x_inter)
             intermediates['pred_x0'] += list(pred)
             return img, intermediates
-        for i, step in enumerate(time_range):
-            index = total_steps - i - 1
-            ts = torch.full((b,), int(step), device=device, dtype=torch.long)
-            if mask is not None:
-                assert x0 is not None
-                img = self._blend_mask(img, mask, x0, ts)
-            img, pred_x0 = self.p_sample_ddim(img, cond, ts, index=index, use_original_steps=ddim_use_original_steps,
-                                              quantize_denoised=quantize_denoised, temperature=temperature,
-                                              noise_dropout=noise_dropout, score_corrector=score_corrector,
-                                              corrector_kwargs=corrector_kwargs,
-                                              unconditional_guidance_scale=unconditional_guidance_scale,
-                                              unconditional_conditioning=unconditional_conditioning, i=i,
-                                              inference_loss=inference_loss, **kwargs)
-            if callback:
-                callback(i)
-            if img_callback:
-                img_callback(pred_x0, i)
-            if index % log_every_t == 0 or index == total_steps - 1:
-                intermediates['x_inter'].append(img)
-                intermediates['pred_x0'].append(pred_x0)
+        announce = getattr(getattr(self.model, 'engine', None), 'set_timestep_schedule', None)
+        if announce is not None:
+            announce([int(step) for step in time_range])
+        try:
+            for i, step in enumerate(time_range):
+                index = total_steps - i - 1
+                ts = torch.full((b,), int(step), device=device, dtype=torch.long)
+                self._t_uniform = (ts, int(step)) if announce is not None else None
+                if mask is not None:
+                    assert x0 is not None
+                    img = self._blend_mask(img, mask, x0, ts)
+                img, pred_x0 = self.p_sample_ddim(img, cond, ts, index=index, use_original_steps=ddim_use_original_steps,
+                                                  quantize_denoised=quantize_denoised, temperature=temperature,
+                                                  noise_dropout=noise_dropout, score_corrector=score_corrector,
+                                                  corrector_kwargs=corrector_kwargs,
+                                                  unconditional_guidance_scale=unconditional_guidance_scale,
+                                                  unconditional_conditioning=unconditional_conditioning, i=i,
+                                                  inference_loss=inference_loss, **kwargs)
+                if callback:
+                    callback(i)
+                if img_callback:
+                    img_callback(pred_x0, i)
+                if index % log_every_t == 0 or index == total_steps - 1:
+                    intermediates['x_inter'].append(img)
+                    intermediates['pred_x0'].append(pred_x0)
+        finally:
+            self._t_uniform = None
         return img, intermediates
 
     def p_sample_ddim(self, x, c, t, index, repeat_noise=False, use_original_steps=False, quantize_denoised=False,
@@ -306,7 +318,7 @@
         uc, scale = unconditional_conditioning, unconditional_guidance_scale
         e_u = None
         if uc is None or scale == 1.:
-            e_c = self.model.apply_model(x, t, c, **kwargs)
+            e_c = self.model.apply_model(x, t, c, **self._t_kw(t, kwargs))
         elif 'composable_diffusion' in kwargs:
             kw = {k: v for k, v in kwargs.items() if k != 'composable_diffusion'}
             n = kwargs['composable_diffusion'] + 1
diff --git a/include/fgdm.h b/include/fgdm.h
--- a/include/fgdm.h
+++ b/include/fgdm.h
@@ -84,6 +84,15 @@
 int fgdm_apply_model(fgdm_engine* e, const float* x, const int64_t* t, const float* t_float, const float* ctx,
                      const float* pcond, const float* control_scales, int B, int H, int W, int flags, float* eps_out,
                      void* stream);
+
+int fgdm_set_timestep_schedule(fgdm_engine* e, const int64_t* timesteps, int S, void* stream);
+int fgdm_apply_model_uniform_t(fgdm_engine* e, const float* x, const int64_t* t, int64_t t_uniform, const float* ctx,
+                               const float* pcond, const float* control_scales, int B, int H, int W, int flags, float* eps_out,
+                               void* stream);
+int fgdm_emb_table_stats(fgdm_engine* e, int64_t* chain_launches, int64_t* table_reads, int32_t* rows);
+int fgdm_embed(fgdm_engine* e, int net, const int64_t* t, int B, float* out, int64_t out_capacity_floats, int32_t* width, void* stream);
+int fgdm_emb_table_read(fgdm_engine* e, int net, float* out, int64_t out_capacity_floats, int32_t* rows, int32_t* width, void* stream);
+int fgdm_emb_plan(const int64_t* timesteps, int S, int64_t* rows, int32_t* row_of, const int64_t* probes, int n_probes, int32_t* probe_rows);
 
 int fgdm_clip_encode(fgdm_engine* e, const int64_t* ids, int B, int T, float* out, void* stream);
 int fgdm_clip_encode_skip(fgdm_engine* e, const int64_t* ids, int B, int T, int clip_skip, float* out, void* stream);
```

Result: no change. 8.183 (median of 6 runs) (+0.4%).
